# NVIDIA/nv-wavenet

Hardware: AMD Instinct MI355X
Metric: samples/sec (all GPUs) in real time (every utterance >= 24 kHz) and max real-time batch @24kHz, R64/S256/A256 20L fp16 (higher is better)
Workload: dtype f16; 1 GPU; C3: R=64 S=256 A=256 L=20 maxDilation=512 fp16, autoregressive generation at steady state (each step = samples 640..895 of every utterance: all dilated taps live, all rings wrapped; the steps re-run that sample range -- same launch, same memory traffic -- so from the second step on the rings hold the previous step's values: a timing workload, not one long utterance); batch_per_gpu=12288, global_batch=12288, parallelism=batch-sharded x1, final RCCL all_gather

## Files before the change

### include/nv_wavenet_c.h

```cpp
#ifndef NV_WAVENET_C_H
#define NV_WAVENET_C_H

#include <stddef.h>

#ifdef __cplusplus
extern "C" {
#endif

typedef struct nvw_engine nvw_engine;

typedef void (*nvw_consume_fn)(int* yOut, int init_sample, int count, void* user);

#define NVW_ABI_VERSION 7
int nvw_abi_version(void);
int nvw_supported(int R, int S, int A, int precision);
int nvw_list_supported(int* out, int max);

nvw_engine* nvw_create(int R, int S, int A, int precision, int num_layers, int max_dilation,
                       int batch_size, int num_samples, int implementation, int tanh_embed);
nvw_engine* nvw_create_ex(int R, int S, int A, int precision, int num_layers, int max_dilation,
                          int batch_size, int num_samples, int implementation, int tanh_embed,
                          int organisation);
void nvw_destroy(nvw_engine* e);

void nvw_set_embeddings(nvw_engine* e, float* embed_prev, float* embed_cur);
void nvw_set_layer_weights(nvw_engine* e, int layer, float* Wprev, float* Wcur, float* Bh,
                           float* Wres, float* Bres, float* Wskip, float* Bskip);
void nvw_set_out_weights(nvw_engine* e, float* Wzs, float* Bzs, float* Wza, float* Bza);
void nvw_set_inputs(nvw_engine* e, float* Lh, float* output_selectors);

void nvw_set_conditioning(nvw_engine* e, float* Lh);
void nvw_set_inputs_n(nvw_engine* e, float* Lh, float* output_selectors, int num_samples);
void nvw_set_conditioning_n(nvw_engine* e, float* Lh, int num_samples);
void nvw_pack_conditioning(nvw_engine* e, float* Lh, int first_sample, int count, void* stream);
void nvw_set_conditioning_direct(nvw_engine* e, float* Lh, int num_samples);
int nvw_set_conditioning_direct_t(nvw_engine* e, const void* Lh, int num_samples, int precision);
void nvw_set_conditioning_packed(nvw_engine* e, const void* frags, int num_samples);
int nvw_set_conditioning_packed_n(nvw_engine* e, const void* frags, int num_samples, size_t elems);
int nvw_cond_tiles(nvw_engine* e);
int nvw_produce_conditioning_f16(const void* x, const void* wfrag, const float* bias, void* out, int tiles, int num_samples,
                                 int num_layers, int kfrags, int nwf, void* stream);
int nvw_max_cond_channels(void);
int nvw_set_conditioning_weights(nvw_engine* e, const float* Wcond, const float* bcond, int n_cond);
int nvw_feature_fragments(nvw_engine* e);
size_t nvw_feature_elems(nvw_engine* e, int num_samples);
int nvw_set_conditioning_features(nvw_engine* e, const void* frags, int num_samples, size_t elems);
int nvw_pack_features(nvw_engine* e, const void* x, int precision, long long b_stride, long long c_stride, long long t_stride,
                      int first_sample, int count, void* stream);
int nvw_set_features(nvw_engine* e, const void* x, int precision, long long b_stride, long long c_stride, long long t_stride,
                     int num_samples);
int nvw_set_upsampling(nvw_engine* e, const float* up_w, const float* up_b, int window, int stride);
int nvw_set_mel(nvw_engine* e, const void* mel, int precision, long long b_stride, long long c_stride, long long f_stride, int frames);
int nvw_upsample_features(nvw_engine* e, int first_sample, int count, void* stream);
int nvw_get_features(nvw_engine* e, void* dst, int first_sample, int count);
int nvw_generate_stream(nvw_engine* e, int num_samples_per_chunk, nvw_consume_fn consume, void* user, int num_samples, int batch_size, int* yOut,
                        void* stream);
void nvw_set_selectors(nvw_engine* e, float* output_selectors, int num_samples);
unsigned nvw_chain_status(nvw_engine* e);
unsigned nvw_chain_fallbacks(nvw_engine* e);
unsigned nvw_chain_last_timeout(nvw_engine* e);
void nvw_set_chain_timeout_ms(nvw_engine* e, double ms);
void nvw_set_clock_probe(nvw_engine* e, int on);
void nvw_set_ring_in_lds(nvw_engine* e, int mode);
double nvw_last_launch_clock_ghz(nvw_engine* e);
int nvw_run_range(nvw_engine* e, int init_sample, int count, int num_samples, int batch_size, void* stream);
void nvw_reset_history(nvw_engine* e, void* stream);
void nvw_set_selector_seed(nvw_engine* e, unsigned long long seed);
void nvw_set_audio_out(nvw_engine* e, short* pcm_out);
void nvw_set_audio_out_n(nvw_engine* e, short* pcm_out, size_t elems);
void nvw_kernel_info(nvw_engine* e, int batch_size, int dump_activations, char* buf, int buf_size);

int nvw_run(nvw_engine* e, int num_samples, int batch_size, int* yOut, int batch_size_per_block,
            int dump_activations, void* stream);
int nvw_run_partial(nvw_engine* e, int init_sample, int num_samples, int batch_size, int* yOut,
                    int batch_size_per_block, int dump_activations, void* stream);
int nvw_run_chunks(nvw_engine* e, int num_samples_per_chunk, nvw_consume_fn consume, void* user,
                   int num_samples, int batch_size, int* yOut, int batch_size_per_block,
                   int dump_activations, void* stream);

void nvw_get_xt_out(nvw_engine* e, int layer, float* dst);
void nvw_get_skip_out(nvw_engine* e, int layer, float* dst);
void nvw_get_zs(nvw_engine* e, float* dst);
void nvw_get_za(nvw_engine* e, float* dst);
void nvw_get_p(nvw_engine* e, float* dst);
void nvw_get_y_out(nvw_engine* e, int* yOut, int offset, int size, void* stream);

int nvw_slots_begin(nvw_engine* e, int window);
int nvw_slot_start(nvw_engine* e, int slot, const void* x, int precision, long long c_stride, long long t_stride, int length,
                   unsigned uid);
int nvw_slot_stop(nvw_engine* e, int slot);
int nvw_slots_step(nvw_engine* e, int count, int* yOut, short* pcm, void* stream);
void nvw_slots_end(nvw_engine* e);

int nvw_slot_start_mel(nvw_engine* e, int slot, const void* mel, int precision, long long c_stride, long long f_stride, int frames,
                       int final, unsigned uid);
int nvw_slot_mel_frames(nvw_engine* e, int slot, int frames, int final);
int nvw_slots_headroom(nvw_engine* e);
int nvw_slots_get_features(nvw_engine* e, void* dst, long long first_sample, int count);

size_t nvw_slot_state_bytes(nvw_engine* e);
int nvw_slot_move(nvw_engine* e, int from, int to);
int nvw_slot_save(nvw_engine* e, int slot, void* dst, void* stream);
int nvw_slot_resume(nvw_engine* e, int slot, const void* state, const void* x, int precision, long long c_stride, long long t_stride,
                    int length);
int nvw_slot_resume_mel(nvw_engine* e, int slot, const void* state, const void* mel, int precision, long long c_stride,
                        long long f_stride, int frames, int final);

typedef struct {
    int slot;
    unsigned uid;
    int done;
    int mel;
} nvw_slot_saved;
int nvw_slots_save_list(nvw_engine* e, const int* slots, int n, void* dst, long long stride, nvw_slot_saved* saved, void* stream);
typedef struct {
    int slot;
    int mel;
    const void* src;
    int precision;
    long long c_stride, t_stride;
    int length;
    int final;
} nvw_slot_resume_req;
int nvw_slots_resume_list(nvw_engine* e, const nvw_slot_resume_req* reqs, int n, const void* states, long long stride);

typedef struct {
    int slot;
    unsigned uid;
    long long first;
    int n;
    int finished;
    long long offset;
} nvw_slot_piece;
long long nvw_slots_step_ragged(nvw_engine* e, int count, int* samples, short* pcm, long long capacity, nvw_slot_piece* pieces,
                                int max_pieces, int* n_pieces, unsigned long long* ticket, void* stream);
int nvw_slots_wait(nvw_engine* e, unsigned long long ticket);
float nvw_slots_time_outputs(nvw_engine* e, int ragged, int count, int* samples, short* pcm, long long capacity, int reps, void* stream);
int nvw_slots_done(nvw_engine* e, unsigned long long ticket);
void* nvw_pinned_alloc(size_t bytes);
void nvw_pinned_free(void* p);

int nvw_set_temperatures(nvw_engine* e, const float* T, int n);
int nvw_slot_set_temperature(nvw_engine* e, int slot, float T);
float nvw_slot_temperature(nvw_engine* e, int slot);

int nvw_set_prime(nvw_engine* e, const int* y, const int* n, int batch, int max_n, long long stride);
// ... 101 lines not shown
```

### nv_wavenet_amd/_lib.py

```python
import ctypes as C
import os

_HERE = os.path.dirname(os.path.abspath(__file__))
LIB_PATH = os.environ.get("NVW_LIB") or os.path.join(_HERE, "libwavenet_infer.so")

if not os.path.exists(LIB_PATH):
    raise ImportError(
        "nv_wavenet_amd: %s is missing. Build it with `python -c 'import __graft_entry__ as g; g.build()'` "
        "or `make -C nv_wavenet_amd/csrc`. There is no CPU fallback for the engine." % LIB_PATH)

import torch

lib = C.CDLL(LIB_PATH)

_fp = C.c_void_p
CONSUME_FN = C.CFUNCTYPE(None, C.c_void_p, C.c_int, C.c_int, C.c_void_p)

SIGNATURES = {
    "nvw_abi_version": (C.c_int, []),
    "nvw_supported": (C.c_int, [C.c_int] * 4),
    "nvw_list_supported": (C.c_int, [C.POINTER(C.c_int), C.c_int]),
    "nvw_create": (C.c_void_p, [C.c_int] * 10),
    "nvw_create_ex": (C.c_void_p, [C.c_int] * 11),
    "nvw_destroy": (None, [C.c_void_p]),
    "nvw_set_embeddings": (None, [C.c_void_p, _fp, _fp]),
    "nvw_set_layer_weights": (None, [C.c_void_p, C.c_int] + [_fp] * 7),
    "nvw_set_out_weights": (None, [C.c_void_p] + [_fp] * 4),
    "nvw_set_inputs": (None, [C.c_void_p, _fp, _fp]),
    "nvw_set_conditioning": (None, [C.c_void_p, _fp]),
    "nvw_set_inputs_n": (None, [C.c_void_p, _fp, _fp, C.c_int]),
    "nvw_set_conditioning_n": (None, [C.c_void_p, _fp, C.c_int]),
    "nvw_pack_conditioning": (None, [C.c_void_p, _fp, C.c_int, C.c_int, C.c_void_p]),
    "nvw_set_conditioning_direct": (None, [C.c_void_p, _fp, C.c_int]),
    "nvw_set_conditioning_direct_t": (C.c_int, [C.c_void_p, _fp, C.c_int, C.c_int]),
    "nvw_set_conditioning_packed": (None, [C.c_void_p, _fp, C.c_int]),
    "nvw_set_conditioning_packed_n": (C.c_int, [C.c_void_p, _fp, C.c_int, C.c_size_t]),
    "nvw_cond_tiles": (C.c_int, [C.c_void_p]),
    "nvw_produce_conditioning_f16": (C.c_int, [_fp, _fp, _fp, _fp, C.c_int, C.c_int, C.c_int, C.c_int, C.c_int, C.c_void_p]),
    "nvw_max_cond_channels": (C.c_int, []),
    "nvw_set_conditioning_weights": (C.c_int, [C.c_void_p, _fp, _fp, C.c_int]),
    "nvw_feature_fragments": (C.c_int, [C.c_void_p]),
    "nvw_feature_elems": (C.c_size_t, [C.c_void_p, C.c_int]),
    "nvw_set_conditioning_features": (C.c_int, [C.c_void_p, _fp, C.c_int, C.c_size_t]),
    "nvw_pack_features": (C.c_int, [C.c_void_p, _fp, C.c_int, C.c_longlong, C.c_longlong, C.c_longlong, C.c_int, C.c_int, C.c_void_p]),
    "nvw_set_features": (C.c_int, [C.c_void_p, _fp, C.c_int, C.c_longlong, C.c_longlong, C.c_longlong, C.c_int]),
    "nvw_set_upsampling": (C.c_int, [C.c_void_p, _fp, _fp, C.c_int, C.c_int]),
    "nvw_set_mel": (C.c_int, [C.c_void_p, _fp, C.c_int, C.c_longlong, C.c_longlong, C.c_longlong, C.c_int]),
    "nvw_upsample_features": (C.c_int, [C.c_void_p, C.c_int, C.c_int, C.c_void_p]),
    "nvw_get_features": (C.c_int, [C.c_void_p, _fp, C.c_int, C.c_int]),
    "nvw_generate_stream": (C.c_int, [C.c_void_p, C.c_int, CONSUME_FN, C.c_void_p, C.c_int, C.c_int, _fp, C.c_void_p]),
    "nvw_set_selectors": (None, [C.c_void_p, _fp, C.c_int]),
    "nvw_chain_status": (C.c_uint, [C.c_void_p]),
    "nvw_chain_fallbacks": (C.c_uint, [C.c_void_p]),
    "nvw_chain_last_timeout": (C.c_uint, [C.c_void_p]),
    "nvw_set_chain_timeout_ms": (None, [C.c_void_p, C.c_double]),
    "nvw_set_clock_probe": (None, [C.c_void_p, C.c_int]),
    "nvw_set_ring_in_lds": (None, [C.c_void_p, C.c_int]),
    "nvw_last_launch_clock_ghz": (C.c_double, [C.c_void_p]),
    "nvw_run_range": (C.c_int, [C.c_void_p, C.c_int, C.c_int, C.c_int, C.c_int, C.c_void_p]),
    "nvw_reset_history": (None, [C.c_void_p, C.c_void_p]),
    "nvw_set_selector_seed": (None, [C.c_void_p, C.c_ulonglong]),
    "nvw_set_audio_out": (None, [C.c_void_p, C.c_void_p]),
    "nvw_set_audio_out_n": (None, [C.c_void_p, C.c_void_p, C.c_size_t]),
    "nvw_kernel_info": (None, [C.c_void_p, C.c_int, C.c_int, C.c_char_p, C.c_int]),
    "nvw_run": (C.c_int, [C.c_void_p, C.c_int, C.c_int, _fp, C.c_int, C.c_int, C.c_void_p]),
    "nvw_run_partial": (C.c_int, [C.c_void_p, C.c_int, C.c_int, C.c_int, _fp, C.c_int, C.c_int, C.c_void_p]),
    "nvw_run_chunks": (C.c_int, [C.c_void_p, C.c_int, CONSUME_FN, C.c_void_p, C.c_int, C.c_int, _fp, C.c_int,
                                 C.c_int, C.c_void_p]),
    "nvw_get_xt_out": (None, [C.c_void_p, C.c_int, _fp]),
    "nvw_get_skip_out": (None, [C.c_void_p, C.c_int, _fp]),
    "nvw_get_zs": (None, [C.c_void_p, _fp]),
    "nvw_get_za": (None, [C.c_void_p, _fp]),
    "nvw_get_p": (None, [C.c_void_p, _fp]),
    "nvw_get_y_out": (None, [C.c_void_p, _fp, C.c_int, C.c_int, C.c_void_p]),
    "nvw_slots_begin": (C.c_int, [C.c_void_p, C.c_int]),
    "nvw_slot_start": (C.c_int, [C.c_void_p, C.c_int, _fp, C.c_int, C.c_longlong, C.c_longlong, C.c_int, C.c_uint]),
    "nvw_slot_stop": (C.c_int, [C.c_void_p, C.c_int]),
    "nvw_slots_step": (C.c_int, [C.c_void_p, C.c_int, _fp, _fp, C.c_void_p]),
    "nvw_slots_end": (None, [C.c_void_p]),
    "nvw_slot_start_mel": (C.c_int, [C.c_void_p, C.c_int, _fp, C.c_int, C.c_longlong, C.c_longlong, C.c_int, C.c_int, C.c_uint]),
    "nvw_slot_mel_frames": (C.c_int, [C.c_void_p, C.c_int, C.c_int, C.c_int]),
    "nvw_slots_headroom": (C.c_int, [C.c_void_p]),
    "nvw_slots_get_features": (C.c_int, [C.c_void_p, _fp, C.c_longlong, C.c_int]),
    "nvw_slot_state_bytes": (C.c_size_t, [C.c_void_p]),
    "nvw_slot_move": (C.c_int, [C.c_void_p, C.c_int, C.c_int]),
    "nvw_slot_save": (C.c_int, [C.c_void_p, C.c_int, _fp, C.c_void_p]),
    "nvw_slot_resume": (C.c_int, [C.c_void_p, C.c_int, _fp, _fp, C.c_int, C.c_longlong, C.c_longlong, C.c_int]),
    "nvw_slot_resume_mel": (C.c_int, [C.c_void_p, C.c_int, _fp, _fp, C.c_int, C.c_longlong, C.c_longlong, C.c_int, C.c_int]),
    "nvw_slots_save_list": (C.c_int, [C.c_void_p, C.c_void_p, C.c_int, _fp, C.c_longlong, C.c_void_p, C.c_void_p]),
    "nvw_slots_resume_list": (C.c_int, [C.c_void_p, C.c_void_p, C.c_int, _fp, C.c_longlong]),
    "nvw_slots_step_ragged": (C.c_longlong, [C.c_void_p, C.c_int, _fp, _fp, C.c_longlong, C.c_void_p, C.c_int, C.POINTER(C.c_int),
                                             C.POINTER(C.c_ulonglong), C.c_void_p]),
    "nvw_slots_time_outputs": (C.c_float, [C.c_void_p, C.c_int, C.c_int, _fp, _fp, C.c_longlong, C.c_int, C.c_void_p]),
    "nvw_slots_wait": (C.c_int, [C.c_void_p, C.c_ulonglong]),
    "nvw_slots_done": (C.c_int, [C.c_void_p, C.c_ulonglong]),
    "nvw_set_temperatures": (C.c_int, [C.c_void_p, _fp, C.c_int]),
    "nvw_slot_set_temperature": (C.c_int, [C.c_void_p, C.c_int, C.c_float]),
    "nvw_slot_temperature": (C.c_float, [C.c_void_p, C.c_int]),
    "nvw_set_prime": (C.c_int, [C.c_void_p, _fp, _fp, C.c_int, C.c_int, C.c_longlong]),
    "nvw_slot_prime": (C.c_int, [C.c_void_p, C.c_int, _fp, C.c_int]),
    "nvw_slot_primed": (C.c_int, [C.c_void_p, C.c_int]),
    "nvw_prefill_window": (C.c_int, [C.c_void_p]),
    "nvw_prefill_states": (C.c_int, [C.c_void_p, C.c_void_p, C.c_int, _fp, C.c_longlong, C.c_void_p]),
    "nvw_score_max_samples": (C.c_int, [C.c_void_p]),
    "nvw_score_samples": (C.c_int, [C.c_void_p, C.c_void_p, C.c_int, C.c_void_p]),
    "nvw_upsample_row_elems": (C.c_int, [C.c_void_p]),
    "nvw_upsample_requests": (C.c_int, [C.c_void_p, C.c_void_p, C.c_int, C.c_void_p]),
    "nvw_prefill_states_mel": (C.c_int, [C.c_void_p, C.c_void_p, C.c_int, _fp, C.c_longlong, C.c_void_p]),
    "nvw_score_samples_mel": (C.c_int, [C.c_void_p, C.c_void_p, C.c_int, C.c_void_p]),
    "nvw_score_chunks": (C.c_int, [C.c_void_p, C.c_void_p, C.c_int, C.c_void_p]),
    "nvw_score_chunks_mel": (C.c_int, [C.c_void_p, C.c_void_p, C.c_int, C.c_void_p]),
    "nvw_pinned_alloc": (C.c_void_p, [C.c_size_t]),
    "nvw_pinned_free": (None, [C.c_void_p]),
    "nvw_device_synchronize": (None, []),
    "nvw_time_runs": (C.c_float, [C.c_void_p, C.c_int, C.c_int, C.c_int, C.c_int, C.c_void_p]),
    "wavenet_infer": (None, [C.c_int, C.c_int, _fp, _fp, C.c_int, C.c_int] + [C.POINTER(C.c_void_p)] * 7 +
                      [_fp, _fp, C.c_int, _fp, C.c_int, _fp]),
    "get_R": (C.c_int, []),
    "get_S": (C.c_int, []),
    "get_A": (C.c_int, []),
}

ABI_VERSION = 7
_abi = getattr(lib, "nvw_abi_version", None)
_have = None
if _abi is not None:
    _abi.restype, _abi.argtypes = C.c_int, []
    _have = _abi()
if _have != ABI_VERSION:
    raise ImportError("nv_wavenet_amd: %s implements revision %s of include/nv_wavenet_c.h, this package expects %d: rebuild it "
                      "(make -C nv_wavenet_amd/csrc)" % (LIB_PATH, "<none: too old>" if _have is None else _have, ABI_VERSION))

for _name, (_res, _args) in SIGNATURES.items():
    _fn = getattr(lib, _name)
    _fn.restype = _res
    _fn.argtypes = _args


def addr(x):
    if x is None:
# ... 11 lines not shown
```

### nv_wavenet_amd/csrc/engine_base.hpp

```cpp
#pragma once
#include "../../include/nv_wavenet_c.h"
#include "nv_wavenet.hpp"

struct nvw_engine {
    virtual ~nvw_engine() {}
    virtual void setEmbeddings(float*, float*) = 0;
    virtual void setLayerWeights(int, float*, float*, float*, float*, float*, float*, float*) = 0;
    virtual void setOutWeights(float*, float*, float*, float*) = 0;
    virtual void setInputs(float*, float*, int) = 0;
    virtual void setConditioning(float*, int) = 0;
    virtual void packConditioning(float*, int, int, hipStream_t) = 0;
    virtual void setConditioningDirect(const void*, int, int) = 0;
    virtual void setConditioningPacked(const void*, int) = 0;
    virtual int condTiles() = 0;
    virtual bool setConditioningWeights(const float*, const float*, int) = 0;
    virtual int featureFragments() = 0;
    virtual size_t featureElems(int) = 0;
    virtual void setConditioningFeatures(const void*, int) = 0;
    virtual void packFeatures(const void*, int, long long, long long, long long, int, int, hipStream_t) = 0;
    virtual void setFeatures(const void*, int, long long, long long, long long, int) = 0;
    virtual int conditioningChannels() = 0;
    virtual bool setUpsampling(const float*, const float*, int, int) = 0;
    virtual int upsamplingStride() = 0;
    virtual int melSamples() = 0;
    virtual bool hasFeatureBuffer() = 0;
    virtual int maxBatch() = 0;
    virtual void getFeatures(void*, int, int) = 0;
    virtual void setMel(const void*, int, long long, long long, long long, int) = 0;
    virtual void upsampleFeatures(int, int, hipStream_t) = 0;
    virtual bool run_stream(int, nvw_consume_fn, void*, int, int, int*, hipStream_t) = 0;
    virtual size_t condPackedElems(int) = 0;
    virtual void setSelectors(float*, int) = 0;
    virtual bool run_range(int, int, int, int, hipStream_t) = 0;
    virtual void resetHistory(hipStream_t) = 0;
    virtual bool supported() = 0;
    virtual unsigned chainStatus() = 0;
    virtual unsigned chainFallbacks() = 0;
    virtual unsigned chainLastTimeout() = 0;
    virtual void setChainTimeoutMs(double) = 0;
    virtual void setClockProbe(bool) = 0;
    virtual void setRingInLds(int) = 0;
    virtual double lastLaunchClockGHz() = 0;
    virtual int precisionBits() = 0;
    virtual int maxSamples() = 0;
    virtual void setSelectorSeed(unsigned long long) = 0;
    virtual void setAudioOut(short*, size_t) = 0;
    virtual void kernelInfo(int, bool, char*, int) = 0;
    virtual bool run(int, int, int*, int, bool, hipStream_t) = 0;
    virtual bool run_partial(int, int, int, int*, int, bool, hipStream_t) = 0;
    virtual bool run_chunks(int, nvw_consume_fn, void*, int, int, int*, int, bool, hipStream_t) = 0;
    virtual void getXtOut(int, float*) = 0;
    virtual void getSkipOut(int, float*) = 0;
    virtual void getZs(float*) = 0;
    virtual void getZa(float*) = 0;
    virtual void getP(float*) = 0;
    virtual void getYOut(int*, int, int, hipStream_t) = 0;
    virtual bool setTemperatures(const float*, int) = 0;
    virtual bool setPrime(const int*, const int*, int, int, long long) = 0;
    virtual int prefillWindow() = 0;
    virtual int prefillStates(const wn::PrefillReq*, int, void*, long long, hipStream_t) = 0;
    virtual int scoreMaxSamples() = 0;
    virtual int scoreSamples(const wn::ScoreReq*, int, hipStream_t) = 0;
    virtual int upsampleRowElems() = 0;
    virtual int upsampleRequests(const wn::MelTimeReq*, int, hipStream_t) = 0;
    virtual int prefillStatesMel(const wn::PrefillMelReq*, int, void*, long long, hipStream_t) = 0;
    virtual int scoreSamplesMel(const wn::ScoreMelReq*, int, hipStream_t) = 0;
    virtual int scoreChunks(const wn::ScoreChunkReq*, int, hipStream_t) = 0;
    virtual int scoreChunksMel(const wn::ScoreChunkMelReq*, int, hipStream_t) = 0;
    virtual wn::SlotSession& slots() = 0;
};
static_assert(sizeof(nvw_slot_piece) == sizeof(wn::SlotPiece) && offsetof(nvw_slot_piece, slot) == offsetof(wn::SlotPiece, slot) &&
              offsetof(nvw_slot_piece, uid) == offsetof(wn::SlotPiece, uid) && offsetof(nvw_slot_piece, finished) == offsetof(wn::SlotPiece, finished) &&
              offsetof(nvw_slot_piece, first) == offsetof(wn::SlotPiece, first) &&
              offsetof(nvw_slot_piece, n) == offsetof(wn::SlotPiece, n) && offsetof(nvw_slot_piece, offset) == offsetof(wn::SlotPiece, offset),
              "nvw_slot_piece is wn::SlotPiece");

static_assert(sizeof(nvw_slot_saved) == sizeof(wn::SlotSaved) && offsetof(nvw_slot_saved, slot) == offsetof(wn::SlotSaved, slot) &&
              offsetof(nvw_slot_saved, uid) == offsetof(wn::SlotSaved, uid) && offsetof(nvw_slot_saved, done) == offsetof(wn::SlotSaved, done) &&
              offsetof(nvw_slot_saved, mel) == offsetof(wn::SlotSaved, mel),
              "nvw_slot_saved is wn::SlotSaved");
static_assert(sizeof(nvw_slot_resume_req) == sizeof(wn::SlotResumeReq) && offsetof(nvw_slot_resume_req, slot) == offsetof(wn::SlotResumeReq, slot) &&
              offsetof(nvw_slot_resume_req, mel) == offsetof(wn::SlotResumeReq, mel) && offsetof(nvw_slot_resume_req, src) == offsetof(wn::SlotResumeReq, src) &&
              offsetof(nvw_slot_resume_req, precision) == offsetof(wn::SlotResumeReq, precision) &&
              offsetof(nvw_slot_resume_req, c_stride) == offsetof(wn::SlotResumeReq, cStride) &&
              offsetof(nvw_slot_resume_req, t_stride) == offsetof(wn::SlotResumeReq, tStride) &&
              offsetof(nvw_slot_resume_req, length) == offsetof(wn::SlotResumeReq, length) &&
              offsetof(nvw_slot_resume_req, final) == offsetof(wn::SlotResumeReq, final),
              "nvw_slot_resume_req is wn::SlotResumeReq");

static_assert(sizeof(nvw_prefill_req) == sizeof(wn::PrefillReq) && offsetof(nvw_prefill_req, y) == offsetof(wn::PrefillReq, y) &&
              offsetof(nvw_prefill_req, n) == offsetof(wn::PrefillReq, n) && offsetof(nvw_prefill_req, x) == offsetof(wn::PrefillReq, x) &&
              offsetof(nvw_prefill_req, precision) == offsetof(wn::PrefillReq, precision) &&
              offsetof(nvw_prefill_req, c_stride) == offsetof(wn::PrefillReq, cStride) &&
              offsetof(nvw_prefill_req, t_stride) == offsetof(wn::PrefillReq, tStride) && offsetof(nvw_prefill_req, uid) == offsetof(wn::PrefillReq, uid) &&
              offsetof(nvw_prefill_req, temperature) == offsetof(wn::PrefillReq, temperature),
              "nvw_prefill_req is wn::PrefillReq");

static_assert(sizeof(nvw_score_req) == sizeof(wn::ScoreReq) && offsetof(nvw_score_req, y) == offsetof(wn::ScoreReq, y) &&
              offsetof(nvw_score_req, n) == offsetof(wn::ScoreReq, n) && offsetof(nvw_score_req, x) == offsetof(wn::ScoreReq, x) &&
              offsetof(nvw_score_req, precision) == offsetof(wn::ScoreReq, precision) &&
              offsetof(nvw_score_req, c_stride) == offsetof(wn::ScoreReq, cStride) &&
              offsetof(nvw_score_req, t_stride) == offsetof(wn::ScoreReq, tStride) &&
              offsetof(nvw_score_req, temperature) == offsetof(wn::ScoreReq, temperature) &&
              offsetof(nvw_score_req, logp) == offsetof(wn::ScoreReq, logp) && offsetof(nvw_score_req, rows) == offsetof(wn::ScoreReq, rows),
              "nvw_score_req is wn::ScoreReq");
static_assert(sizeof(nvw_upsample_req) == sizeof(wn::MelTimeReq) && offsetof(nvw_upsample_req, mel) == offsetof(wn::MelTimeReq, mel) &&
              offsetof(nvw_upsample_req, precision) == offsetof(wn::MelTimeReq, precision) &&
              offsetof(nvw_upsample_req, c_stride) == offsetof(wn::MelTimeReq, cStride) &&
              offsetof(nvw_upsample_req, f_stride) == offsetof(wn::MelTimeReq, fStride) &&
              offsetof(nvw_upsample_req, frames) == offsetof(wn::MelTimeReq, frames) &&
              offsetof(nvw_upsample_req, first_sample) == offsetof(wn::MelTimeReq, first) &&
              offsetof(nvw_upsample_req, count) == offsetof(wn::MelTimeReq, count) && offsetof(nvw_upsample_req, dst) == offsetof(wn::MelTimeReq, dst),
              "nvw_upsample_req is wn::MelTimeReq");
static_assert(sizeof(nvw_prefill_mel_req) == sizeof(wn::PrefillMelReq) && offsetof(nvw_prefill_mel_req, y) == offsetof(wn::PrefillMelReq, y) &&
              offsetof(nvw_prefill_mel_req, n) == offsetof(wn::PrefillMelReq, n) && offsetof(nvw_prefill_mel_req, mel) == offsetof(wn::PrefillMelReq, mel) &&
              offsetof(nvw_prefill_mel_req, precision) == offsetof(wn::PrefillMelReq, precision) &&
              offsetof(nvw_prefill_mel_req, c_stride) == offsetof(wn::PrefillMelReq, cStride) &&
              offsetof(nvw_prefill_mel_req, f_stride) == offsetof(wn::PrefillMelReq, fStride) &&
              offsetof(nvw_prefill_mel_req, frames) == offsetof(wn::PrefillMelReq, frames) &&
              offsetof(nvw_prefill_mel_req, uid) == offsetof(wn::PrefillMelReq, uid) &&
              offsetof(nvw_prefill_mel_req, temperature) == offsetof(wn::PrefillMelReq, temperature),
              "nvw_prefill_mel_req is wn::PrefillMelReq");
static_assert(sizeof(nvw_score_mel_req) == sizeof(wn::ScoreMelReq) && offsetof(nvw_score_mel_req, y) == offsetof(wn::ScoreMelReq, y) &&
              offsetof(nvw_score_mel_req, n) == offsetof(wn::ScoreMelReq, n) && offsetof(nvw_score_mel_req, mel) == offsetof(wn::ScoreMelReq, mel) &&
              offsetof(nvw_score_mel_req, precision) == offsetof(wn::ScoreMelReq, precision) &&
              offsetof(nvw_score_mel_req, c_stride) == offsetof(wn::ScoreMelReq, cStride) &&
              offsetof(nvw_score_mel_req, f_stride) == offsetof(wn::ScoreMelReq, fStride) &&
              offsetof(nvw_score_mel_req, frames) == offsetof(wn::ScoreMelReq, frames) &&
              offsetof(nvw_score_mel_req, temperature) == offsetof(wn::ScoreMelReq, temperature) &&
              offsetof(nvw_score_mel_req, logp) == offsetof(wn::ScoreMelReq, logp) && offsetof(nvw_score_mel_req, rows) == offsetof(wn::ScoreMelReq, rows),
              "nvw_score_mel_req is wn::ScoreMelReq");
static_assert(sizeof(nvw_score_chunk_req) == sizeof(wn::ScoreChunkReq) && offsetof(nvw_score_chunk_req, state) == offsetof(wn::ScoreChunkReq, state) &&
              offsetof(nvw_score_chunk_req, y) == offsetof(wn::ScoreChunkReq, y) && offsetof(nvw_score_chunk_req, n) == offsetof(wn::ScoreChunkReq, n) &&
              offsetof(nvw_score_chunk_req, x) == offsetof(wn::ScoreChunkReq, x) &&
              offsetof(nvw_score_chunk_req, precision) == offsetof(wn::ScoreChunkReq, precision) &&
              offsetof(nvw_score_chunk_req, c_stride) == offsetof(wn::ScoreChunkReq, cStride) &&
              offsetof(nvw_score_chunk_req, t_stride) == offsetof(wn::ScoreChunkReq, tStride) &&
              offsetof(nvw_score_chunk_req, uid) == offsetof(wn::ScoreChunkReq, uid) &&
              offsetof(nvw_score_chunk_req, temperature) == offsetof(wn::ScoreChunkReq, temperature) &&
              offsetof(nvw_score_chunk_req, logp) == offsetof(wn::ScoreChunkReq, logp) &&
              offsetof(nvw_score_chunk_req, rows) == offsetof(wn::ScoreChunkReq, rows) &&
              offsetof(nvw_score_chunk_req, state_out) == offsetof(wn::ScoreChunkReq, stateOut),
              "nvw_score_chunk_req is wn::ScoreChunkReq");
static_assert(sizeof(nvw_score_chunk_mel_req) == sizeof(wn::ScoreChunkMelReq) &&
              offsetof(nvw_score_chunk_mel_req, state) == offsetof(wn::ScoreChunkMelReq, state) &&
              offsetof(nvw_score_chunk_mel_req, y) == offsetof(wn::ScoreChunkMelReq, y) &&
              offsetof(nvw_score_chunk_mel_req, n) == offsetof(wn::ScoreChunkMelReq, n) &&
              offsetof(nvw_score_chunk_mel_req, mel) == offsetof(wn::ScoreChunkMelReq, mel) &&
              offsetof(nvw_score_chunk_mel_req, precision) == offsetof(wn::ScoreChunkMelReq, precision) &&
              offsetof(nvw_score_chunk_mel_req, c_stride) == offsetof(wn::ScoreChunkMelReq, cStride) &&
              offsetof(nvw_score_chunk_mel_req, f_stride) == offsetof(wn::ScoreChunkMelReq, fStride) &&
              offsetof(nvw_score_chunk_mel_req, frames) == offsetof(wn::ScoreChunkMelReq, frames) &&
              offsetof(nvw_score_chunk_mel_req, uid) == offsetof(wn::ScoreChunkMelReq, uid) &&
              offsetof(nvw_score_chunk_mel_req, temperature) == offsetof(wn::ScoreChunkMelReq, temperature) &&
              offsetof(nvw_score_chunk_mel_req, logp) == offsetof(wn::ScoreChunkMelReq, logp) &&
              offsetof(nvw_score_chunk_mel_req, rows) == offsetof(wn::ScoreChunkMelReq, rows) &&
              offsetof(nvw_score_chunk_mel_req, state_out) == offsetof(wn::ScoreChunkMelReq, stateOut),
              "nvw_score_chunk_mel_req is wn::ScoreChunkMelReq");

template <typename Tw, typename Td, int R, int S, int A>
struct EngineImpl : nvw_engine {
    nvWavenetInfer<Tw, Td, R, S, A> eng;
    int cap;
    EngineImpl(int L, int maxD, int B, int N, int impl, bool tanhEmbed, int org) : eng(L, maxD, B, N, impl, tanhEmbed, org), cap(N) {}
    void setEmbeddings(float* p, float* c) override { eng.setEmbeddings(p, c); }
    void setLayerWeights(int l, float* a, float* b, float* c, float* d, float* e, float* f, float* g) override {
        eng.setLayerWeights(l, a, b, c, d, e, f, g);
    }
    void setOutWeights(float* a, float* b, float* c, float* d) override { eng.setOutWeights(a, b, c, d); }
    void setInputs(float* Lh, float* sel, int n) override { eng.setInputs(Lh, sel, n); }
    void setConditioning(float* Lh, int n) override { eng.setConditioning(Lh, n); }
    void packConditioning(float* Lh, int first, int count, hipStream_t s) override { eng.packConditioning(Lh, first, count, s); }
    void setConditioningDirect(const void* Lh, int n, int prec) override { eng.setConditioningDirect(Lh, n, prec); }
    void setConditioningPacked(const void* frags, int n) override { eng.setConditioningPacked(frags, n); }
    int condTiles() override { return eng.condTiles(); }
    bool setConditioningWeights(const float* W, const float* b, int n) override { return eng.setConditioningWeights(W, b, n); }
    int featureFragments() override { return eng.featureFragments(); }
    size_t featureElems(int n) override { return eng.featureElems(n); }
    void setConditioningFeatures(const void* f, int n) override { eng.setConditioningFeatures(f, n); }
    void packFeatures(const void* x, int prec, long long bS, long long cS, long long tS, int first, int count, hipStream_t s) override {
        eng.packFeatures(x, prec, bS, cS, tS, first, count, s);
    }
    void setFeatures(const void* x, int prec, long long bS, long long cS, long long tS, int n) override { eng.setFeatures(x, prec, bS, cS, tS, n); }
    int conditioningChannels() override { return eng.conditioningChannels(); }
    bool setUpsampling(const float* W, const float* b, int window, int stride) override { return eng.setUpsampling(W, b, window, stride); }
    int upsamplingStride() override { return eng.upsamplingStride(); }
    int melSamples() override { return eng.melSamples(); }
    bool hasFeatureBuffer() override { return eng.hasFeatureBuffer(); }
    int maxBatch() override { return eng.maxBatch(); }
    void getFeatures(void* d, int first, int count) override { eng.getFeatures(d, first, count); }
    void setMel(const void* mel, int prec, long long bS, long long cS, long long fS, int frames) override { eng.setMel(mel, prec, bS, cS, fS, frames); }
    void upsampleFeatures(int first, int count, hipStream_t s) override { eng.upsampleFeatures(first, count, s); }
    bool run_stream(int chunk, nvw_consume_fn fn, void* user, int n, int b, int* y, hipStream_t s) override {
        return eng.run_stream(chunk, [fn, user](int* yo, int i, int c) { if (fn) fn(yo, i, c, user); }, n, b, y, s);
    }
    size_t condPackedElems(int n) override { return eng.condPackedElems(n); }
    void setSelectors(float* sel, int n) override { eng.setSelectors(sel, n); }
    bool run_range(int i, int c, int n, int b, hipStream_t s) override { return eng.run_range(i, c, n, b, s); }
    void resetHistory(hipStream_t s) override { eng.resetHistory(s); }
    bool supported() override { return eng.supported(); }
    unsigned chainStatus() override { return eng.chainStatus(); }
    unsigned chainFallbacks() override { return eng.chainFallbacks(); }
    unsigned chainLastTimeout() override { return eng.chainLastTimeout(); }
    void setChainTimeoutMs(double ms) override { eng.setChainTimeoutMs(ms); }
    void setClockProbe(bool on) override { eng.setClockProbe(on); }
    void setRingInLds(int mode) override { eng.setRingInLds(mode); }
    double lastLaunchClockGHz() override { return eng.lastLaunchClockGHz(); }
    int precisionBits() override { return std::is_same<Td, float>::value ? 32 : 16; }
    int maxSamples() override { return cap; }
    void setSelectorSeed(unsigned long long seed) override { eng.setSelectorSeed(seed); }
    void setAudioOut(short* pcm, size_t n) override { eng.setAudioOut(pcm, n); }
    void kernelInfo(int b, bool dump, char* buf, int n) override { eng.kernelInfo(b, dump, buf, n); }
    bool run(int n, int b, int* y, int bspb, bool dump, hipStream_t s) override {
        return eng.run(n, b, y, bspb, dump, s);
    }
    bool run_partial(int i, int n, int b, int* y, int bspb, bool dump, hipStream_t s) override {
        return eng.run_partial(i, n, b, y, bspb, dump, s);
    }
    bool run_chunks(int chunk, nvw_consume_fn fn, void* user, int n, int b, int* y, int bspb, bool dump,
                    hipStream_t s) override {
        return eng.run_chunks(chunk, [fn, user](int* yo, int i, int c) { if (fn) fn(yo, i, c, user); }, n, b, y,
                              bspb, dump, s);
    }
    void getXtOut(int l, float* d) override { eng.getXtOut(l, d); }
    void getSkipOut(int l, float* d) override { eng.getSkipOut(l, d); }
    void getZs(float* d) override { eng.getZs(d); }
    void getZa(float* d) override { eng.getZa(d); }
    void getP(float* d) override { eng.getP(d); }
    void getYOut(int* y, int off, int size, hipStream_t s) override { eng.getYOut(y, off, size, s); }
    bool setTemperatures(const float* T, int n) override { return eng.setTemperatures(T, n); }
    bool setPrime(const int* y, const int* n, int batch, int maxN, long long stride) override { return eng.setPrime(y, n, batch, maxN, stride); }
    int prefillWindow() override { return eng.prefillWindow(); }
    int prefillStates(const wn::PrefillReq* reqs, int count, void* dst, long long stride, hipStream_t s) override {
        return eng.prefillStates(reqs, count, dst, stride, s);
    }
    int scoreMaxSamples() override { return eng.scoreMaxSamples(); }
    int scoreSamples(const wn::ScoreReq* reqs, int count, hipStream_t s) override { return eng.scoreSamples(reqs, count, s); }
    int upsampleRowElems() override { return eng.upsampleRowElems(); }
    int upsampleRequests(const wn::MelTimeReq* reqs, int count, hipStream_t s) override { return eng.upsampleRequests(reqs, count, s); }
    int prefillStatesMel(const wn::PrefillMelReq* reqs, int count, void* dst, long long stride, hipStream_t s) override {
        return eng.prefillStatesMel(reqs, count, dst, stride, s);
    }
    int scoreSamplesMel(const wn::ScoreMelReq* reqs, int count, hipStream_t s) override { return eng.scoreSamplesMel(reqs, count, s); }
    int scoreChunks(const wn::ScoreChunkReq* reqs, int count, hipStream_t s) override { return eng.scoreChunks(reqs, count, s); }
    int scoreChunksMel(const wn::ScoreChunkMelReq* reqs, int count, hipStream_t s) override { return eng.scoreChunksMel(reqs, count, s); }
    wn::SlotSession& slots() override { return eng.slots(); }
};

typedef nvw_engine* (*nvw_factory_fn)(int L, int maxD, int B, int N, int impl, int tanhEmbed, int organisation);

#define WN_CAT2(a, b) a##b
#define WN_CAT(a, b) WN_CAT2(a, b)
#define WN_FACTORY_NAME(R, S, A, P) WN_CAT(WN_CAT(WN_CAT(WN_CAT(WN_CAT(WN_CAT(WN_CAT(nvw_make_, R), _), S), _), A), _p), P)
```

### nv_wavenet_amd/csrc/nv_wavenet.hpp

```cpp
#pragma once

#include <assert.h>
#include <hip/hip_fp16.h>
#include <hip/hip_runtime.h>
#include <stdio.h>
#include <stdlib.h>
#include <string.h>

#include <cmath>
#include <memory>
#include <type_traits>
#include <vector>

#include "gpu_check.hpp"
#include "mel_time.hpp"
#include "prefill.hpp"
#include "score.hpp"
#include "score_carry.hpp"
#include "slots_session.hpp"
#include "wn_chain.hpp"
#include "wn_kernels.hpp"

enum nvwOrganisation {
    NVW_ORG_AUTO = 0,
    NVW_ORG_WG = 1,
    NVW_ORG_WG1 = 2,
    NVW_ORG_WG2 = 3,
    NVW_ORG_WG3 = 4,
    NVW_ORG_CHAIN = 5,
    NVW_ORG_CHAIN1 = 6,
    NVW_ORG_RETIRED7 = 7,
    NVW_ORG_RETIRED8 = 8,
    NVW_ORG_RETIRED9 = 9,
    NVW_ORG_WG4 = 10,
    NVW_ORG_LAST = NVW_ORG_WG4
};

template <typename T_weight, typename T_data, int R = 64, int S = 128, int A = 256>
class nvWavenetInfer : protected wn::SlotHost {
public:
    enum Implementation { AUTO = 0, SINGLE_BLOCK, DUAL_BLOCK, PERSISTENT, MANYBLOCK_NONPERSISTENT };

    static constexpr bool F16 = !std::is_same<T_data, float>::value;
    static_assert(std::is_same<T_data, float>::value || std::is_same<T_data, half>::value,
                  "T_data must be float or half");
    static_assert(std::is_same<T_weight, float>::value == std::is_same<T_data, float>::value,
                  "T_weight/T_data must be <float,float> or <half2,half>");

protected:
    using C = wn::Cfg<F16, R, S, A, 1>;
    using CC = wn::CCfg<F16, R, S, A>;
    using elem = typename wn::Prec<F16>::elem;
    static constexpr int KFC = wn::feat_kfc<F16>();
    static constexpr int KC = KFC * 16 * wn::Prec<F16>::TPF;
    using CF = wn::Cfg<F16, R, S, A, 1, KFC>;
    static_assert(wn::kSoftScaleUnit == wn::kLog2e, "T = 1 is the kernel's default scale");

    Implementation m_implementation;
    int m_numLayers, m_maxBatch, m_maxSamples, m_maxDilation, m_tiles, m_numCUs;
    int m_org;
    bool m_supported;
    int m_chainLpc, m_chainStages;
    bool m_tanhEmbed;
    int m_num_samples_per_chunk;
    int m_ringSlots;
    int m_ringDirtyTiles;
    int m_ringLdsMode;
    int m_lastStride;

    elem* m_wblob;
    float* m_bias;
    elem* m_embedPrev;
    elem* m_embedCur;
    elem* m_cond;
    int m_condRawSamples;
    const void* m_condRaw;
    int m_condRawKind;
    const void* m_condUser;
    int m_condUserSamples;
    elem* m_wblobF;
    float* m_biasF;
    float* m_condW;
    float* m_condB;
    int2* m_restream;
    int m_restreamN;
    int m_nCond;
    bool m_featDirty;
    elem* m_upTab;
    float* m_upBias;
    int m_upWindow, m_upStride;
    elem* m_melFrag;
    int m_melFrames, m_melCap;
    elem* m_feat;
    const void* m_featPtr;
    int m_featSamples;
    float* m_outputSelectors;
    elem* m_ring;
    int *m_yInPrev, *m_yInCur, *m_yOut;
    float *m_XtOut, *m_skipOut, *m_Zs, *m_Za, *m_p;
    unsigned long long* m_mail;
    unsigned* m_chainStatus;
    size_t m_mailBytes;
    elem* m_ringShadow;
    int* m_histShadow;
    long long m_chainTimeoutTicks;

    float* m_stage;
    size_t m_stageElems;

    bool m_useRng;
    unsigned long long m_rngSeed;
    short* m_pcm;
    short* m_mulaw;
    short* m_pcmUser;
    size_t m_pcmUserElems;
    unsigned long long* m_clk;
    bool m_clkOn;

    wn::TemperatureTable m_temps;
    wn::PrimeTable m_prime;
    wn::Score m_score;
    wn::MelTime m_melTime;
    wn::Prefill m_prefill;
    std::unique_ptr<wn::SlotSession> m_slots;

    std::vector<hipEvent_t> m_poolEvents;
    hipEvent_t pooledEvent(size_t i) {
        while (m_poolEvents.size() <= i) {
            hipEvent_t ev;
            gpuErrChk(hipEventCreateWithFlags(&ev, hipEventDisableTiming));
            m_poolEvents.push_back(ev);
        }
        return m_poolEvents[i];
    }
    static bool isDevicePtr(const void* ptr) { return wn::is_device_ptr(ptr); }
    size_t m_stageUsed;
    void stageBegin(size_t totalElems) {
        if (totalElems > m_stageElems) {
            gpuErrChk(hipStreamSynchronize(0));
            if (m_stage) gpuErrChk(hipFree(m_stage));
            gpuErrChk(hipMalloc(&m_stage, totalElems * sizeof(float)));
            m_stageElems = totalElems;
        }
        m_stageUsed = 0;
    }
    const float* onDevice(const float* src, size_t n) {
        if (isDevicePtr(src)) return src;
        assert(m_stageUsed + n <= m_stageElems);
        float* d = m_stage + m_stageUsed;
        m_stageUsed += (n + 3) & ~(size_t)3;
        gpuErrChk(hipMemcpyAsync(d, src, n * sizeof(float), hipMemcpyHostToDevice, 0));
        return d;
    }
    static int gridFor(size_t n) {
        size_t g = (n + 255) / 256;
        return (int)(g > 4096 ? 4096 : (g ? g : 1));
    }
    void packWeight(size_t blockFrag, const float* src, int M, int K, int gateRT) {
        const float* d = onDevice(src, (size_t)M * K);
        hipLaunchKernelGGL((wn::pack_weight_kernel<F16>), dim3(gridFor((size_t)M * K)), dim3(256), 0, 0,
                           m_wblob + blockFrag * C::FRAG_ELEMS, d, M, K, C::NW,
                           C::waveStreamFrags(m_numLayers) * C::FRAG_ELEMS, gateRT);
        gpuErrChk(hipGetLastError());
    }
    void convertTo(elem* dst, const float* src, size_t n) {
        const float* d = onDevice(src, n);
        hipLaunchKernelGGL((wn::convert_kernel<F16>), dim3(gridFor(n)), dim3(256), 0, 0, dst, d, n);
        gpuErrChk(hipGetLastError());
    }
    template <int BT> static size_t ldsNeed(int L, int embTables, bool dump = true) { return wn::Cfg<F16, R, S, A, BT>::ldsBytes(L, embTables, dump); }
    static constexpr size_t kLdsMax = 160 * 1024;
    template <int BT> bool ldsFits(bool dump = true) const { return ldsNeed<BT>(m_numLayers, 0, dump) <= kLdsMax; }
    template <int BT> int embTables(bool dump = true) const {
        return ldsNeed<BT>(m_numLayers, 2, dump) <= kLdsMax ? 2 : ldsNeed<BT>(m_numLayers, 1, dump) <= kLdsMax ? 1 : 0;
    }
    void fillSchedule(wn::Params& p) const {
        int d = 1, off = 0;
        for (int l = 0; l < m_numLayers; l++) {
            p.dil[l].d = d;
            p.dil[l].off = off;
            p.dil[l].lds = 0;
            off += d;
            d <<= 1;
            if (d > m_maxDilation) d = 1;
        }
        p.dil[m_numLayers] = p.dil[0];
        p.dil[m_numLayers + 1] = p.dil[1];
    }
    template <int BT> size_t placeLdsRing(wn::Params& p, size_t need) const {
        using CB = wn::Cfg<F16, R, S, A, BT>;
        int D = 0;
        for (int d = 1; d <= m_maxDilation && d <= WN_LDS_RING_MAXD; d <<= 1)
            if (need + (size_t)CB::ringTailSlots(CB::ldsRingSlots(m_numLayers, m_maxDilation, d)) * CB::RING_SLOT <= kLdsMax) D = d;
        p.ldsRingD = D;
        int slot = 0;
        for (int l = 0; l < m_numLayers; l++) {
            p.dil[l].lds = slot;
            if (p.dil[l].d <= D) slot += p.dil[l].d;
        }
        p.dil[m_numLayers] = p.dil[0];
        p.dil[m_numLayers + 1] = p.dil[1];
        return (size_t)CB::ringTailSlots(slot) * CB::RING_SLOT;
    }
    static constexpr bool lrBuilt(bool dump, int raw) { return !dump && (raw == 0 || F16); }
    template <int BT> size_t ringPlan(wn::Params& p, size_t need, bool dump, int raw) const {
        p.ldsRingD = 0;
#ifdef WN_EXP_TWO_WG
        if (BT == 1) return 0;
#endif
        if (!lrBuilt(dump, raw) || m_ringLdsMode < 0) return 0;
        wn::Params q = p;
        const size_t bytes = placeLdsRing<BT>(q, need);
        if (q.ldsRingD <= 0) return 0;
        p = q;
        return bytes;
    }
    template <int BT, bool EMB, bool DUMP, int RAW> bool launchK(wn::Params& p, int tiles, int nEmb, hipStream_t stream) {
        using CB = wn::Cfg<F16, R, S, A, BT>;
        const int grid = (tiles + BT - 1) / BT;
        p.embLds = nEmb;
        const size_t need = ldsNeed<BT>(m_numLayers, nEmb, DUMP);
        if constexpr (lrBuilt(DUMP, RAW)) {
            const size_t ringBytes = ringPlan<BT>(p, need, DUMP, RAW);
            if (p.ldsRingD > 0) {
                hipLaunchKernelGGL((wn::wavenet_wg<F16, R, S, A, BT, EMB, DUMP, RAW, true>), dim3(grid), dim3(CB::THREADS), need + ringBytes, stream, p);
                return hipGetLastError() == hipSuccess;
            }
        }
        p.ldsRingD = 0;
        hipLaunchKernelGGL((wn::wavenet_wg<F16, R, S, A, BT, EMB, DUMP, RAW>), dim3(grid), dim3(CB::THREADS), need, stream, p);
        return hipGetLastError() == hipSuccess;
    }
    template <int BT> int planEmb(bool dump, int raw) const {
        int nEmb = embTables<BT>(dump);
#ifdef WN_EXP_TWO_WG
        if (BT == 1) return 0;
#endif
        if (nEmb == 2 && m_ringLdsMode >= 0 && lrBuilt(dump, raw)) {
            wn::Params q;
            fillSchedule(q);
            placeLdsRing<BT>(q, ldsNeed<BT>(m_numLayers, 2, dump));
            const int D2 = q.ldsRingD;
            placeLdsRing<BT>(q, ldsNeed<BT>(m_numLayers, 1, dump));
            if (D2 == 0 || (D2 < 2 && q.ldsRingD > D2)) nEmb = 1;
        }
        return nEmb;
    }
    template <int BT, bool DUMP, int RAW> bool launchE(wn::Params& p, int tiles, hipStream_t stream) {
        const int nEmb = planEmb<BT>(DUMP, RAW);
        return nEmb ? launchK<BT, true, DUMP, RAW>(p, tiles, nEmb, stream) : launchK<BT, false, DUMP, RAW>(p, tiles, 0, stream);
    }
    template <int BT, bool DUMP> bool launchD(wn::Params& p, int tiles, hipStream_t stream) {
        if (p.condRawKind == 3) return launchE<BT, DUMP, 3>(p, tiles, stream);
        if constexpr (F16) {
            if (p.condRawKind == 2) return launchE<BT, DUMP, 2>(p, tiles, stream);
        }
        return p.condRawKind == 1 ? launchE<BT, DUMP, 1>(p, tiles, stream) : launchE<BT, DUMP, 0>(p, tiles, stream);
    }
    template <int BT> bool launch(wn::Params& p, int tiles, hipStream_t stream) {
        if (!p.dump) {
            if constexpr (F16) return launchD<BT, false>(p, tiles, stream);
            else if (p.condRawKind == 0) return launchE<BT, false, 0>(p, tiles, stream);
        }
        return launchD<BT, true>(p, tiles, stream);
    }
    template <int BT, bool EMB, bool DUMP, int RAW> void allowLdsK() {
        const size_t need = ldsNeed<BT>(m_numLayers, EMB ? embTables<BT>(DUMP) : 0, DUMP);
        if (need <= kLdsMax) {
            gpuErrChk(hipFuncSetAttribute((const void*)wn::wavenet_wg<F16, R, S, A, BT, EMB, DUMP, RAW>,
                                          hipFuncAttributeMaxDynamicSharedMemorySize, (int)need));
            if constexpr (lrBuilt(DUMP, RAW))
                gpuErrChk(hipFuncSetAttribute((const void*)wn::wavenet_wg<F16, R, S, A, BT, EMB, DUMP, RAW, true>,
                                              hipFuncAttributeMaxDynamicSharedMemorySize, (int)kLdsMax));
        }
    }
    template <int BT, bool DUMP> void allowLdsD() {
        allowLdsK<BT, false, DUMP, 0>();
        allowLdsK<BT, true, DUMP, 0>();
        allowLdsK<BT, false, DUMP, 1>();
        allowLdsK<BT, true, DUMP, 1>();
        allowLdsK<BT, false, DUMP, 3>();
        allowLdsK<BT, true, DUMP, 3>();
        if constexpr (F16) {
            allowLdsK<BT, false, DUMP, 2>();
            allowLdsK<BT, true, DUMP, 2>();
        }
    }
    template <int BT> void allowLds() {
        allowLdsD<BT, true>();
        if constexpr (F16) allowLdsD<BT, false>();
        else {
            allowLdsK<BT, false, false, 0>();
            allowLdsK<BT, true, false, 0>();
        }
    }
    float* headBias() { return m_bias + (size_t)m_numLayers * C::BIAS_L; }

    static int chainStagesFor(int L, int lpc) { return (L + lpc - 1) / lpc + 1; }
    static int chainLpcMax(int L) {
        if (!CC::SUPPORTED) return 0;
        const int ns = (L + CC::LPC - 1) / CC::LPC;
        return (L + ns - 1) / ns;
    }
    bool chainFits(int lpc, int tiles) const {
        return lpc > 0 && chainStagesFor(m_numLayers, lpc) * ((tiles + CC::TPC_MAX - 1) / CC::TPC_MAX) <= m_numCUs;
    }
    int singleOrg(int) const { return NVW_ORG_WG; }
    struct OrgTimes {
        static constexpr double kClockMHz = 2390.0;
        static constexpr double kStreamBytesPerClk = 58.0;
        static constexpr double kStreamLayerUs = 0.25;
        static constexpr double kHeadUs = 4.0;
        static constexpr double kChainHopUs = 1.1;
        static constexpr double kChainLayerUs(int r) { return r >= 128 ? 0.55 : 0.4; }
        static constexpr double kChainUnitUs = 5.0;
    };
    int pickOrganisation(int tiles) const {
        const int single = singleOrg(tiles);
        const int lpc = chainLpcMax(m_numLayers);
        if (!chainFits(lpc, tiles)) return single;
        const double wBytes = sizeof(elem) * ((double)m_numLayers * (5.0 * R * R + (double)S * R) + (double)A * S + (double)A * A);
        const int wgMax = WG3 ? 3 : WG2 ? 2 : 1;
        const int rounds = (tiles + wgMax * m_numCUs - 1) / (wgMax * m_numCUs);
        const double tStream = (wBytes / (OrgTimes::kStreamBytesPerClk * OrgTimes::kClockMHz) + OrgTimes::kStreamLayerUs * m_numLayers + OrgTimes::kHeadUs) * rounds;
        const int stages = chainStagesFor(m_numLayers, lpc), perLaunch = m_numCUs / stages;
        const int tpc = (tiles + perLaunch - 1) / perLaunch;
        if (tpc > 1 && WG3) return single;
        double tChain = OrgTimes::kChainHopUs * stages + OrgTimes::kChainLayerUs(R) * m_numLayers + OrgTimes::kHeadUs;
        if (tpc * OrgTimes::kChainUnitUs > tChain) tChain = tpc * OrgTimes::kChainUnitUs;
        const double tWg = tiles > m_numCUs ? tStream * (tiles > 2 * m_numCUs && WG3 ? 1.9 : WG2 ? 1.4 : 1.0) : tStream;
        return tChain < tWg ? NVW_ORG_CHAIN : single;
    }
    void resolveOrganisation(int requested) {
        const int tiles = (m_maxBatch + 15) / 16;
        int org = requested;
        if (org == NVW_ORG_AUTO) {
            switch (m_implementation) {
                case SINGLE_BLOCK: org = singleOrg(tiles); break;
                case DUAL_BLOCK:
                case PERSISTENT: org = chainFits(chainLpcMax(m_numLayers), tiles) ? NVW_ORG_CHAIN : singleOrg(tiles); break;
                case MANYBLOCK_NONPERSISTENT:
                    org = (CC::SUPPORTED && chainFits(1, tiles)) ? NVW_ORG_CHAIN1
                          : chainFits(chainLpcMax(m_numLayers), tiles) ? NVW_ORG_CHAIN : singleOrg(tiles);
                    break;
                default: org = pickOrganisation(tiles); break;
            }
        }
        if (org == NVW_ORG_CHAIN && !chainFits(chainLpcMax(m_numLayers), tiles)) org = singleOrg(tiles);
        if (org == NVW_ORG_CHAIN1 && !(CC::SUPPORTED && chainFits(1, tiles))) org = singleOrg(tiles);
        m_org = org;
        m_chainLpc = org == NVW_ORG_CHAIN ? chainLpcMax(m_numLayers) : org == NVW_ORG_CHAIN1 ? 1 : 0;
        m_chainStages = m_chainLpc ? chainStagesFor(m_numLayers, m_chainLpc) : 0;
    }
    bool isChain() const { return m_chainLpc > 0; }
    static constexpr bool kChainHoistBuilt = F16 && CC::SUPPORTED && CC::LP <= 2 && A <= 512;
    static bool chainHoists(int tpc) { return kChainHoistBuilt && tpc > WN_CHAIN_HOIST_FROM; }
    int chainTpc(int tiles) const {
        const int perLaunch = m_numCUs / (m_chainStages > 0 ? m_chainStages : 1);
        int tpc = perLaunch > 0 ? (tiles + perLaunch - 1) / perLaunch : 1;
#ifdef WN_CHAIN_TPC_MIN
        if (tpc < WN_CHAIN_TPC_MIN) tpc = WN_CHAIN_TPC_MIN;
#endif
        return tpc < 1 ? 1 : tpc > CC::TPC_MAX ? CC::TPC_MAX : tpc;
    }
    static constexpr bool WG3 = F16 && R <= 64;
    static constexpr bool WG2 = R < 128;
    bool wg3Fits() const {
        if constexpr (WG3) return ldsFits<3>();
        return false;
    }
    static constexpr bool WG4 = WG3;
    bool wg4Fits() const {
        if constexpr (WG4) return ldsFits<4>(false);
        return false;
    }
    int wgTiles(int tiles) const {
#ifdef WN_EXP_TWO_WG
        if (m_org == NVW_ORG_WG && tiles <= 2 * m_numCUs) return 1;
#endif
        bool four = m_org == NVW_ORG_WG4;
        if (m_org == NVW_ORG_WG && tiles > WN_WG4_FROM * m_numCUs) {
            const int r4 = (tiles + 4 * m_numCUs - 1) / (4 * m_numCUs), r3 = (tiles + 3 * m_numCUs - 1) / (3 * m_numCUs);
            four = r4 * 47 <= r3 * 36;
        }
        if (four && wg4Fits() && wg3Fits()) return 4;
        const bool three = four || m_org == NVW_ORG_WG3 || (m_org == NVW_ORG_WG && tiles > 2 * m_numCUs);
        if (three && wg3Fits()) return 3;
        const bool two = three || m_org == NVW_ORG_WG2 || (m_org == NVW_ORG_WG && tiles > m_numCUs);
        if constexpr (WG2) return (two && ldsFits<2>()) ? 2 : 1;
        return 1;
    }

public:
    nvWavenetInfer(int numLayers, int maxDilation, int batchSize, int numSamples, int impl = 0,
                   bool tanhEmbed = true, int organisation = NVW_ORG_AUTO)
        : m_implementation((Implementation)impl), m_numLayers(numLayers), m_maxBatch(batchSize),
          m_maxSamples(numSamples), m_maxDilation(maxDilation), m_tanhEmbed(tanhEmbed),
          m_num_samples_per_chunk(0), m_lastStride(numSamples), m_cond(NULL), m_condRawSamples(0), m_condRaw(NULL), m_condRawKind(0), m_condUser(NULL), m_condUserSamples(0),
          m_wblobF(NULL), m_biasF(NULL), m_condW(NULL), m_condB(NULL), m_restream(NULL), m_restreamN(0), m_nCond(0), m_featDirty(true),
          m_upTab(NULL), m_upBias(NULL), m_upWindow(0), m_upStride(0), m_melFrag(NULL), m_melFrames(0), m_melCap(0),
          m_feat(NULL), m_featPtr(NULL), m_featSamples(0),
          m_mail(NULL), m_chainStatus(NULL), m_mailBytes(0), m_ringShadow(NULL), m_histShadow(NULL),
          m_chainTimeoutTicks(wn::kChainTimeoutTicks), m_stage(NULL), m_stageElems(0), m_useRng(false), m_rngSeed(0), m_pcm(NULL),
          m_mulaw(NULL), m_pcmUser(NULL), m_pcmUserElems(0), m_clk(NULL), m_clkOn(false), m_temps(batchSize), m_prime(batchSize), m_stageUsed(0) {
        assert(numLayers >= 2 && batchSize > 0 && numSamples > 0 && maxDilation > 0);
        m_ringDirtyTiles = 0;
        m_ringLdsMode = 0;
        assert(numLayers <= wn::kMaxLayers);
        {
            int dev = 0;
            hipDeviceProp_t prop;
            gpuErrChk(hipGetDevice(&dev));
            gpuErrChk(hipGetDeviceProperties(&prop, dev));
            m_numCUs = prop.multiProcessorCount;
        }
        resolveOrganisation(organisation);
        m_supported = isChain() || ldsFits<1>();
        if (!m_supported)
            fprintf(stderr, "nvWavenetInfer: R=%d S=%d A=%d with %d layers needs %zu bytes of LDS (> 160 KiB): unsupported\n", R,
                    S, A, numLayers, ldsNeed<1>(numLayers, 0));

        {
            const int tiles = (batchSize + 15) / 16;
            int group = isChain() ? 1 : wgTiles(tiles);
            if (group >= 3 && wg4Fits()) group = 12;
            m_tiles = (tiles + group - 1) / group * group;
        }

        {
            int d = 1, slots = 0;
            for (int l = 0; l < numLayers; l++) {
                slots += d;
                d <<= 1;
                if (d > maxDilation) d = 1;
            }
            m_ringSlots = slots;
        }

        const size_t wElems = (size_t)C::NW * C::waveStreamFrags(numLayers) * C::FRAG_ELEMS;
        gpuErrChk(hipMalloc(&m_wblob, wElems * sizeof(elem)));
        gpuErrChk(hipMemset(m_wblob, 0, wElems * sizeof(elem)));
        const size_t bElems = (size_t)numLayers * C::BIAS_L + 2 * A;
        gpuErrChk(hipMalloc(&m_bias, bElems * sizeof(float)));
        gpuErrChk(hipMemset(m_bias, 0, bElems * sizeof(float)));
        gpuErrChk(hipMalloc(&m_embedPrev, (size_t)A * R * sizeof(elem)));
        gpuErrChk(hipMalloc(&m_embedCur, (size_t)A * R * sizeof(elem)));
        gpuErrChk(hipMemset(m_embedPrev, 0, (size_t)A * R * sizeof(elem)));
        gpuErrChk(hipMemset(m_embedCur, 0, (size_t)A * R * sizeof(elem)));

        gpuErrChk(hipMalloc(&m_outputSelectors, (size_t)numSamples * batchSize * sizeof(float)));
        gpuErrChk(hipMemset(m_outputSelectors, 0, (size_t)numSamples * batchSize * sizeof(float)));

        const size_t ringBytes = ringElems() * sizeof(elem);
        gpuErrChk(hipMalloc(&m_ring, ringBytes));
        gpuErrChk(hipMemset(m_ring, 0, ringBytes));

        gpuErrChk(hipMalloc(&m_yInPrev, batchSize * sizeof(int)));
        gpuErrChk(hipMalloc(&m_yInCur, batchSize * sizeof(int)));
        gpuErrChk(hipMalloc(&m_yOut, (size_t)numSamples * batchSize * sizeof(int)));
        gpuErrChk(hipMemset(m_yOut, 0, (size_t)numSamples * batchSize * sizeof(int)));

        gpuErrChk(hipMalloc(&m_XtOut, (size_t)numLayers * R * batchSize * sizeof(float)));
        gpuErrChk(hipMalloc(&m_skipOut, (size_t)numLayers * S * batchSize * sizeof(float)));
        gpuErrChk(hipMalloc(&m_Zs, (size_t)A * batchSize * sizeof(float)));
        gpuErrChk(hipMalloc(&m_Za, (size_t)A * batchSize * sizeof(float)));
        gpuErrChk(hipMalloc(&m_p, (size_t)A * batchSize * sizeof(float)));
        gpuErrChk(hipMemset(m_XtOut, 0, (size_t)numLayers * R * batchSize * sizeof(float)));
        gpuErrChk(hipMemset(m_skipOut, 0, (size_t)numLayers * S * batchSize * sizeof(float)));
        gpuErrChk(hipMemset(m_Zs, 0, (size_t)A * batchSize * sizeof(float)));
        gpuErrChk(hipMemset(m_Za, 0, (size_t)A * batchSize * sizeof(float)));
        gpuErrChk(hipMemset(m_p, 0, (size_t)A * batchSize * sizeof(float)));

        gpuErrChk(hipMalloc(&m_chainStatus, 4 * sizeof(unsigned)));
        gpuErrChk(hipMemset(m_chainStatus, 0, 4 * sizeof(unsigned)));
        if (isChain()) {
            {
                const int tiles = (batchSize + 15) / 16, perLaunch = m_numCUs / m_chainStages;
                m_mailBytes = CC::mailGranules(tiles < perLaunch ? tiles : perLaunch, m_chainStages, chainTpc(tiles)) * sizeof(unsigned long long);
            }
            gpuErrChk(hipMalloc(&m_mail, m_mailBytes));
            gpuErrChk(hipMemset(m_mail, 0, m_mailBytes));
            gpuErrChk(hipFuncSetAttribute((const void*)wn::wavenet_chain<F16, R, S, A, true>,
                                          hipFuncAttributeMaxDynamicSharedMemorySize, (int)CC::ldsBytes()));
            gpuErrChk(hipFuncSetAttribute((const void*)wn::wavenet_chain<F16, R, S, A, false>,
                                          hipFuncAttributeMaxDynamicSharedMemorySize, (int)CC::ldsBytes()));
            if constexpr (kChainHoistBuilt)
                gpuErrChk(hipFuncSetAttribute((const void*)wn::wavenet_chain<F16, R, S, A, false, true>,
                                              hipFuncAttributeMaxDynamicSharedMemorySize, (int)CC::ldsBytes()));
            if (chainHasFallback()) {
                gpuErrChk(hipMalloc(&m_ringShadow, ringBytes));
// ... 4 lines not shown
        hipLaunchKernelGGL(wn::silence_kernel, dim3(1), dim3(256), 0, 0, m_yInPrev, m_yInCur, m_maxBatch);
        gpuErrChk(hipGetLastError());

        if (ldsFits<1>()) {
            allowLds<1>();
            if (!isChain()) {
                if constexpr (WG2) allowLds<2>();
                if constexpr (WG3) allowLds<3>();
                if constexpr (WG4) {
                    if (wg4Fits()) {
                        allowLdsK<4, false, false, 0>();
                        allowLdsK<4, true, false, 0>();
                    }
                }
            }
        }
        gpuErrChk(hipDeviceSynchronize());
        m_slots.reset(new wn::SlotSession(wn::SlotFacts{m_maxBatch, m_tiles, m_numLayers, m_maxDilation, m_ringSlots, (int)(R * 16 * sizeof(elem) / 1024), R,
                                                        F16, featureElems(1), m_supported, m_ring, m_yInPrev, m_yInCur, A},
                                          *this, m_temps));
    }

    virtual ~nvWavenetInfer() {
        gpuErrChk(hipDeviceSynchronize());
        m_slots.reset();
        for (hipEvent_t ev : m_poolEvents) gpuErrChk(hipEventDestroy(ev));
        gpuErrChk(hipFree(m_wblob));
        gpuErrChk(hipFree(m_bias));
        gpuErrChk(hipFree(m_embedPrev));
        gpuErrChk(hipFree(m_embedCur));
        if (m_cond) gpuErrChk(hipFree(m_cond));
        if (m_wblobF) gpuErrChk(hipFree(m_wblobF));
        if (m_biasF) gpuErrChk(hipFree(m_biasF));
        if (m_condW) gpuErrChk(hipFree(m_condW));
        if (m_condB) gpuErrChk(hipFree(m_condB));
        if (m_restream) gpuErrChk(hipFree(m_restream));
        if (m_feat) gpuErrChk(hipFree(m_feat));
        if (m_upTab) gpuErrChk(hipFree(m_upTab));
        if (m_upBias) gpuErrChk(hipFree(m_upBias));
        if (m_melFrag) gpuErrChk(hipFree(m_melFrag));
        gpuErrChk(hipFree(m_outputSelectors));
        gpuErrChk(hipFree(m_ring));
        gpuErrChk(hipFree(m_yInPrev));
        gpuErrChk(hipFree(m_yInCur));
        gpuErrChk(hipFree(m_yOut));
        gpuErrChk(hipFree(m_XtOut));
        gpuErrChk(hipFree(m_skipOut));
        gpuErrChk(hipFree(m_Zs));
        gpuErrChk(hipFree(m_Za));
        gpuErrChk(hipFree(m_p));
        gpuErrChk(hipFree(m_chainStatus));
        if (m_mail) gpuErrChk(hipFree(m_mail));
        if (m_ringShadow) gpuErrChk(hipFree(m_ringShadow));
        if (m_histShadow) gpuErrChk(hipFree(m_histShadow));
        if (m_stage) gpuErrChk(hipFree(m_stage));
        if (m_pcm) gpuErrChk(hipFree(m_pcm));
        if (m_mulaw) gpuErrChk(hipFree(m_mulaw));
        if (m_clk) gpuErrChk(hipFree(m_clk));
    }

    bool supported() const { return m_supported; }
    unsigned chainStatus() { return statusWord(0); }
    unsigned chainFallbacks() { return statusWord(2); }
    unsigned chainLastTimeout() { return statusWord(1); }
    void setClockProbe(bool on) {
        if (on && !m_clk) {
            gpuErrChk(hipMalloc(&m_clk, 4 * sizeof(unsigned long long)));
            gpuErrChk(hipMemset(m_clk, 0, 4 * sizeof(unsigned long long)));
        }
        m_clkOn = on;
    }
    double lastLaunchClockGHz() {
        if (!m_clk) return 0.0;
        unsigned long long c[4];
        gpuErrChk(hipDeviceSynchronize());
        gpuErrChk(hipMemcpy(c, m_clk, sizeof(c), hipMemcpyDeviceToHost));
        int dev = 0, wallKHz = 0;
        gpuErrChk(hipGetDevice(&dev));
        gpuErrChk(hipDeviceGetAttribute(&wallKHz, hipDeviceAttributeWallClockRate, dev));
        if (c[3] <= c[1] || wallKHz <= 0) return 0.0;
        return (double)(c[2] - c[0]) / (double)(c[3] - c[1]) * (double)wallKHz * 1e-6;
    }
    void setRingInLds(int mode) { m_ringLdsMode = mode < 0 ? -1 : 0; }
    void setChainTimeoutMs(double ms) { m_chainTimeoutTicks = (long long)(ms * 1e5); }

    virtual void setEmbeddings(float* embedPrev, float* embedCur) {
        stageBegin((size_t)2 * A * R);
        convertTo(m_embedPrev, embedPrev, (size_t)A * R);
        convertTo(m_embedCur, embedCur, (size_t)A * R);
        gpuErrChk(hipStreamSynchronize(0));
    }
    bool setConditioningWeights(const float* Wcond, const float* bcond, int nCond) {
        if (nCond <= 0 || nCond > wn::kCondChannelsMax) return false;
        const size_t nW = (size_t)m_numLayers * 2 * R * nCond, nB = (size_t)m_numLayers * 2 * R;
        stageBegin(nW + nB + 8);
        if (!m_condW) {
            gpuErrChk(hipMalloc(&m_condW, (size_t)m_numLayers * KC * 2 * R * sizeof(float)));
            gpuErrChk(hipMalloc(&m_condB, nB * sizeof(float)));
        }
        gpuErrChk(hipMemsetAsync(m_condW, 0, (size_t)m_numLayers * KC * 2 * R * sizeof(float), 0));
        const float* dW = onDevice(Wcond, nW);
        hipLaunchKernelGGL(wn::cond_weight_arrange_kernel, dim3(gridFor(nW)), dim3(256), 0, 0, m_condW, dW, m_numLayers, 2 * R, nCond, KC);
        gpuErrChk(hipGetLastError());
        gpuErrChk(hipMemcpyAsync(m_condB, bcond, nB * sizeof(float), hipMemcpyDefault, 0));
        gpuErrChk(hipStreamSynchronize(0));
        if (nCond != m_nCond) {
            m_upStride = 0;
            m_upWindow = 0;
            m_melFrames = 0;
        }
        m_nCond = nCond;
        m_featDirty = true;
        return true;
    }
    int conditioningChannels() const { return m_nCond; }
    int featureFragments() const { return KFC; }
    size_t featureElems(int numSamples) const { return (size_t)numSamples * m_tiles * KFC * C::FRAG_ELEMS; }
    void setConditioningFeatures(const void* frags, int numSamples) {
        assert(numSamples > 0 && numSamples <= m_maxSamples && m_nCond > 0);
        assert(isDevicePtr(frags));
        resetHistory(0);
        gpuErrChk(hipStreamSynchronize(0));
        dropLhConditioning();
        m_featPtr = frags;
        m_featSamples = numSamples;
    }
    void packFeatures(const void* x, int precision, long long bStride, long long cStride, long long tStride, int firstSample, int count,
                      hipStream_t stream = 0) {
        assert(firstSample >= 0 && count > 0 && firstSample + count <= m_maxSamples && m_nCond > 0);
        assert(precision == 32 || precision == 16);
        assert(isDevicePtr(x));
        if (!m_feat) {
            gpuErrChk(hipMalloc(&m_feat, featureElems(m_maxSamples) * sizeof(elem)));
            gpuErrChk(hipMemsetAsync(m_feat, 0, featureElems(m_maxSamples) * sizeof(elem), stream));
            gpuErrChk(hipStreamSynchronize(stream));
        }
        dropLhConditioning();
        m_featPtr = m_feat;
        m_featSamples = m_maxSamples;
        const int tilesUsed = (m_maxBatch + 15) / 16;
        const size_t nblk = (size_t)tilesUsed * ((count + 7) / 8);
        hipLaunchKernelGGL((wn::pack_features_kernel<F16>), dim3((unsigned)(nblk > 65536 ? 65536 : nblk)), dim3(256), 0, stream,
                           m_feat + featureElems(firstSample), x, precision, bStride, cStride, tStride, m_nCond, m_maxBatch, count, m_tiles,
                           tilesUsed);
        gpuErrChk(hipGetLastError());
    }
    void setFeatures(const void* x, int precision, long long bStride, long long cStride, long long tStride, int numSamples) {
        resetHistory(0);
        packFeatures(x, precision, bStride, cStride, tStride, 0, numSamples, 0);
        gpuErrChk(hipStreamSynchronize(0));
    }
    bool conditioningFromFeatures() const { return m_featPtr != NULL; }
    static constexpr int kUpMaxTaps = 5;
    bool setUpsampling(const float* upW, const float* upB, int window, int stride) {
        if (m_nCond <= 0 || stride <= 0 || window < stride || window % stride != 0 || window / stride > kUpMaxTaps) return false;
        const size_t nW = (size_t)m_nCond * m_nCond * window;
        stageBegin(nW + 128);
        if (m_upTab) gpuErrChk(hipFree(m_upTab));
        const size_t tabElems = (size_t)stride * wn::kUpRowTiles * (window / stride) * KFC * C::FRAG_ELEMS;
        gpuErrChk(hipMalloc(&m_upTab, tabElems * sizeof(elem)));
        if (!m_upBias) gpuErrChk(hipMalloc(&m_upBias, wn::kUpRowTiles * 16 * sizeof(float)));
        gpuErrChk(hipMemsetAsync(m_upBias, 0, wn::kUpRowTiles * 16 * sizeof(float), 0));
        const float* dW = onDevice(upW, nW);
        hipLaunchKernelGGL((wn::pack_upsample_kernel<F16>), dim3(gridFor(tabElems)), dim3(256), 0, 0, m_upTab, dW, m_nCond, window, stride);
        gpuErrChk(hipGetLastError());
        gpuErrChk(hipMemcpyAsync(m_upBias, upB, m_nCond * sizeof(float), hipMemcpyDefault, 0));
// ... 216 lines not shown
    }
    void setSelectorSeed(unsigned long long seed) {
        m_useRng = true;
        m_rngSeed = seed;
    }
    void setAudioOut(short* pcmOut, size_t pcmElems = 0) {
        m_pcmUser = pcmOut;
        m_pcmUserElems = pcmOut ? pcmElems : 0;
        if (pcmOut && !m_pcm) {
            gpuErrChk(hipMalloc(&m_pcm, (size_t)m_maxSamples * m_maxBatch * sizeof(short)));
            gpuErrChk(hipMemset(m_pcm, 0, (size_t)m_maxSamples * m_maxBatch * sizeof(short)));
            ensureMulaw();
        }
    }
    void ensureMulaw() {
        if (!m_mulaw) {
            std::vector<short> table(A);
            const double mu = (double)A - 1.0;
            for (int y = 0; y < A; y++) {
                const double signal = 2.0 * ((double)y / mu) - 1.0;
                const double magnitude = (1.0 / mu) * (std::pow(1.0 + mu, std::fabs(signal)) - 1.0);
                const double v = 32768.0 * (signal > 0 ? magnitude : (signal < 0 ? -magnitude : 0.0));
                table[y] = (short)(int)v;
            }
            gpuErrChk(hipMalloc(&m_mulaw, A * sizeof(short)));
            gpuErrChk(hipMemcpy(m_mulaw, table.data(), A * sizeof(short), hipMemcpyHostToDevice));
        }
    }
    void getAudioOut(short* pcm, int offset, int size, hipStream_t stream = 0) {
        gpuErrChk(hipMemcpy2DAsync(pcm + offset, m_lastStride * sizeof(short), m_pcm + offset,
                                   m_lastStride * sizeof(short), size * sizeof(short), m_maxBatch, hipMemcpyDefault,
                                   stream));
    }

    void kernelInfo(int batch_size, bool dumpActivations, char* buf, int n) const {
        const int tiles = (batch_size + 15) / 16;
        const bool feat = m_featPtr != NULL || m_slots->active();
        const bool chainLaunch = isChain() && !feat;
        const bool dump = dumpActivations || (!F16 && !chainLaunch && (feat || m_condRaw));
        if (chainLaunch) {
            const int perLaunch = m_numCUs / m_chainStages, chains = tiles < perLaunch ? tiles : perLaunch;
            const int tpcNow = chainTpc((m_maxBatch + 15) / 16);
            snprintf(buf, n, "wn::wavenet_chain<%s,%d,%d,%d,DUMP=%d%s> stages=%d layers/stage=%d chains=%d tiles/chain=%d wgs=%d lds=%zu",
                     F16 ? "fp16" : "fp32", R, S, A, dump ? 1 : 0, (!dump && chainHoists(tpcNow)) ? ",HOIST=1" : "", m_chainStages, m_chainLpc, chains, tpcNow,
                     m_chainStages * chains, CC::ldsBytes());
            return;
        }
        const int raw = feat ? 3 : m_condRaw ? m_condRawKind : 0;
        const int bt = launchTiles(tiles, dump, raw);
        int nEmb = planEmb<1>(dump, raw);
        size_t lds = ldsNeed<1>(m_numLayers, nEmb, dump);
        if constexpr (WG2) {
            if (bt == 2) {
                nEmb = planEmb<2>(dump, raw);
                lds = ldsNeed<2>(m_numLayers, nEmb, dump);
            }
        }
        if constexpr (WG3) {
            if (bt == 3) {
                nEmb = planEmb<3>(dump, raw);
                lds = ldsNeed<3>(m_numLayers, nEmb, dump);
            }
            if (bt == 4) {
                nEmb = planEmb<4>(dump, raw);
                lds = ldsNeed<4>(m_numLayers, nEmb, dump);
            }
        }
        int ringD = 0;
        {
            wn::Params q;
            fillSchedule(q);
            size_t rb = 0;
            if (bt == 1) rb = ringPlan<1>(q, lds, dump, raw);
            if constexpr (WG2) {
                if (bt == 2) rb = ringPlan<2>(q, lds, dump, raw);
            }
            if constexpr (WG3) {
                if (bt == 3) rb = ringPlan<3>(q, lds, dump, raw);
                if (bt == 4) rb = ringPlan<4>(q, lds, dump, raw);
            }
            lds += rb;
            ringD = q.ldsRingD;
        }
        char ring[48] = "";
        if (ringD > 0) snprintf(ring, sizeof(ring), " ring_in_lds=d<=%d", ringD);
        snprintf(buf, n, "wn::wavenet_wg<%s,%d,%d,%d,BT=%d,EMBLDS=%d,DUMP=%d,RAW=%d%s> tiles/wg=%d wgs=%d lds=%zu%s",
                 F16 ? "fp16" : "fp32", R, S, A, bt, nEmb, dump ? 1 : 0, raw, ringD > 0 ? ",LR=1" : "", bt, (tiles + bt - 1) / bt, lds, ring);
    }

    void getXtOut(int layer, float* hXt) {
        gpuErrChk(hipMemcpy(hXt, m_XtOut + (size_t)layer * m_maxBatch * R, (size_t)m_maxBatch * R * sizeof(float),
                            hipMemcpyDefault));
    }
    void getSkipOut(int layer, float* hSkipOut) {
        gpuErrChk(hipMemcpy(hSkipOut, m_skipOut + (size_t)layer * m_maxBatch * S,
                            (size_t)m_maxBatch * S * sizeof(float), hipMemcpyDefault));
    }
    void getZs(float* hZs) { gpuErrChk(hipMemcpy(hZs, m_Zs, (size_t)m_maxBatch * A * sizeof(float), hipMemcpyDefault)); }
    void getZa(float* hZa) { gpuErrChk(hipMemcpy(hZa, m_Za, (size_t)m_maxBatch * A * sizeof(float), hipMemcpyDefault)); }
    void getP(float* hP) { gpuErrChk(hipMemcpy(hP, m_p, (size_t)m_maxBatch * A * sizeof(float), hipMemcpyDefault)); }
    void getYOut(int* yOut, int offset, int size, hipStream_t stream = 0) {
        const size_t rowBytes = (size_t)m_lastStride * sizeof(int);
        gpuErrChk(hipMemcpy2DAsync(yOut + offset, rowBytes, m_yOut + offset, rowBytes, (size_t)size * sizeof(int),
                                   (size_t)m_maxBatch, hipMemcpyDefault, stream));
    }

    bool setTemperatures(const float* T, int n) {
        if (m_slots->active()) return false;
        if (T != NULL) {
            if (n < 1 || n > m_maxBatch) return false;
            for (int b = 0; b < n; b++)
                if (!wn::temperature_ok(T[b])) return false;
        }
        gpuErrChk(hipDeviceSynchronize());
        m_temps.reset(false);
        if (T == NULL) return true;
        for (int b = 0; b < n; b++) m_temps.set(b, T[b]);
        m_temps.upload();
        return true;
    }
    float temperature(int b) const { return m_temps.get(b); }

    bool setPrime(const int* y, const int* n, int batch, int maxN, long long stride) {
        if (m_slots->active()) return false;
        if (y == NULL) {
            gpuErrChk(hipDeviceSynchronize());
            m_prime.clear();
            return true;
        }
        if (n == NULL || batch < 1 || batch > m_maxBatch || maxN < 0 || maxN > m_maxSamples || stride < maxN) return false;
        for (int b = 0; b < batch; b++)
            if (n[b] < 0 || n[b] > maxN) return false;
        if (!isDevicePtr(y))
            for (int b = 0; b < batch; b++)
                for (int k = 0; k < n[b]; k++)
                    if (y[b * stride + k] < 0 || y[b * stride + k] >= A) return false;
        m_prime.set(y, n, batch, maxN, stride, m_maxSamples);
        return true;
    }
    int prefillWindow() const { return m_nCond > 0 ? wn::prefill_window(m_ringSlots) : 0; }
    int prefillStates(const wn::PrefillReq* reqs, int count, void* dst, long long stride, hipStream_t stream = 0) {
        if (m_nCond <= 0 || !m_supported) return 0;
        wn::PrefillModel m = prefillModel();
        if (m_featDirty) buildFeatStream(stream);
        m.wblob = m_wblobF;
        m.bias = m_biasF;
        return m_prefill.run(m, reqs, count, dst, stride, stream) ? count : 0;
    }
    wn::PrefillModel prefillModel() const {
        const int L = m_numLayers;
        wn::PrefillModel m;
        m.f16 = F16;
        m.R = R;
        m.A = A;
        m.numLayers = L;
        m.maxDilation = m_maxDilation;
        m.ringSlots = m_ringSlots;
        m.nCond = m_nCond;
        m.tanhEmbed = m_tanhEmbed ? 1 : 0;
        m.wblob = NULL;
        m.waveStreamFrags = CF::waveStreamFrags(L);
        m.bias = NULL;
        m.biasL = C::BIAS_L;
        m.embPrev = m_embedPrev;
        m.embCur = m_embedCur;
        for (int l = 0, d = 1, off = 0; l < L; l++) {
            int dN = d << 1;
            if (dN > m_maxDilation) dN = 1;
// ... 537 lines not shown
```

### nv_wavenet_amd/csrc/wavenet_capi.hip

```cpp
#include <stdlib.h>

#include <vector>

#include "../../include/wavenet_infer.h"
#include "engine_base.hpp"

#define X(R, S, A, P) nvw_engine* WN_FACTORY_NAME(R, S, A, P)(int, int, int, int, int, int, int);
WN_INSTANCES
#undef X

namespace {
struct Entry { int R, S, A, P; nvw_factory_fn make; };
#define X(R, S, A, P) {R, S, A, P, WN_FACTORY_NAME(R, S, A, P)},
const Entry kEntries[] = {WN_INSTANCES};
#undef X
const int kNumEntries = sizeof(kEntries) / sizeof(kEntries[0]);

const Entry* findEntry(int R, int S, int A, int P) {
    for (int i = 0; i < kNumEntries; i++)
        if (kEntries[i].R == R && kEntries[i].S == S && kEntries[i].A == A && kEntries[i].P == P) return &kEntries[i];
    return NULL;
}
}

// ... 119 lines not shown
        fprintf(stderr, "nvw_set_conditioning_features: %zu elements cannot hold %d samples of feature fragments (%zu needed)\n", elems,
                num_samples, e->featureElems(num_samples));
        return 0;
    }
    e->setConditioningFeatures(frags, num_samples);
    return 1;
}
int nvw_pack_features(nvw_engine* e, const void* x, int precision, long long b_stride, long long c_stride, long long t_stride,
                      int first_sample, int count, void* stream) {
    if (!featArgsOk(e, "nvw_pack_features", x, first_sample, count) || (precision != 32 && precision != 16)) return 0;
    e->packFeatures(x, precision, b_stride, c_stride, t_stride, first_sample, count, (hipStream_t)stream);
    return 1;
}
int nvw_set_upsampling(nvw_engine* e, const float* up_w, const float* up_b, int window, int stride) {
    if (!e->setUpsampling(up_w, up_b, window, stride)) {
        fprintf(stderr, "nvw_set_upsampling: window %d / stride %d (a multiple of the stride, at most 5 strides; nvw_set_conditioning_weights first)\n",
                window, stride);
        return 0;
    }
    return 1;
}
int nvw_set_mel(nvw_engine* e, const void* mel, int precision, long long b_stride, long long c_stride, long long f_stride, int frames) {
    const int stride = e->upsamplingStride();
    if (stride <= 0 || !wn::is_device_ptr(mel) || (precision != 32 && precision != 16) || frames <= 0 || (long long)frames * stride > e->maxSamples()) {
        fprintf(stderr, "nvw_set_mel: refused (nvw_set_upsampling first; device memory; 16- or 32-bit floats; frames * stride <= the engine's %d samples)\n",
                e->maxSamples());
        return 0;
    }
    e->setMel(mel, precision, b_stride, c_stride, f_stride, frames);
    return 1;
}
int nvw_upsample_features(nvw_engine* e, int first_sample, int count, void* stream) {
    if (e->upsamplingStride() <= 0 || e->melSamples() <= 0) {
        fprintf(stderr, "nvw_upsample_features: refused (nvw_set_upsampling and nvw_set_mel first)\n");
        return 0;
    }
    if (first_sample < 0 || count <= 0 || (long long)first_sample + count > e->melSamples()) {
        fprintf(stderr, "nvw_upsample_features: samples [%d, %lld) outside the %d the mel frames upsample to\n", first_sample,
                (long long)first_sample + count, e->melSamples());
        return 0;
    }
    e->upsampleFeatures(first_sample, count, (hipStream_t)stream);
    return 1;
}
int nvw_get_features(nvw_engine* e, void* dst, int first_sample, int count) {
    if (!e->hasFeatureBuffer() || dst == NULL || first_sample < 0 || count <= 0 || (long long)first_sample + count > e->maxSamples()) {
        fprintf(stderr, "nvw_get_features: refused (no features packed or upsampled by this engine yet, or samples [%d, %lld) outside its %d)\n",
                first_sample, (long long)first_sample + count, e->maxSamples());
        return 0;
    }
    e->getFeatures(dst, first_sample, count);
    return 1;
}
int nvw_generate_stream(nvw_engine* e, int num_samples_per_chunk, nvw_consume_fn consume, void* user, int num_samples, int batch_size, int* yOut,
                        void* stream) {
    if (e->upsamplingStride() <= 0 || e->melSamples() <= 0) {
        fprintf(stderr, "nvw_generate_stream: refused (nvw_set_upsampling and nvw_set_mel first)\n");
        return 0;
    }
    if (num_samples_per_chunk <= 0 || num_samples <= 0 || num_samples > e->melSamples() || num_samples > e->maxSamples()) {
        fprintf(stderr, "nvw_generate_stream: %d samples in chunks of %d: the mel frames upsample to %d, the engine holds %d\n", num_samples,
                num_samples_per_chunk, e->melSamples(), e->maxSamples());
        return 0;
    }
    if (batch_size <= 0 || batch_size > e->maxBatch()) {
        fprintf(stderr, "nvw_generate_stream: batch %d outside 1..%d\n", batch_size, e->maxBatch());
        return 0;
    }
    return e->run_stream(num_samples_per_chunk, consume, user, num_samples, batch_size, yOut, (hipStream_t)stream) ? 1 : 0;
}
int nvw_set_features(nvw_engine* e, const void* x, int precision, long long b_stride, long long c_stride, long long t_stride,
                     int num_samples) {
    if (!featArgsOk(e, "nvw_set_features", x, 0, num_samples) || (precision != 32 && precision != 16)) return 0;
    e->setFeatures(x, precision, b_stride, c_stride, t_stride, num_samples);
    return 1;
}
void nvw_set_selectors(nvw_engine* e, float* sel, int num_samples) { e->setSelectors(sel, num_samples); }
unsigned nvw_chain_status(nvw_engine* e) { return e->chainStatus(); }
unsigned nvw_chain_fallbacks(nvw_engine* e) { return e->chainFallbacks(); }
unsigned nvw_chain_last_timeout(nvw_engine* e) { return e->chainLastTimeout(); }
void nvw_set_chain_timeout_ms(nvw_engine* e, double ms) { e->setChainTimeoutMs(ms); }
void nvw_set_clock_probe(nvw_engine* e, int on) { e->setClockProbe(on != 0); }
void nvw_set_ring_in_lds(nvw_engine* e, int mode) { e->setRingInLds(mode); }
double nvw_last_launch_clock_ghz(nvw_engine* e) { return e->lastLaunchClockGHz(); }
int nvw_run_range(nvw_engine* e, int init_sample, int count, int num_samples, int batch_size, void* stream) {
    return e->run_range(init_sample, count, num_samples, batch_size, (hipStream_t)stream) ? 1 : 0;
}
void nvw_reset_history(nvw_engine* e, void* stream) { e->resetHistory((hipStream_t)stream); }
void nvw_set_selector_seed(nvw_engine* e, unsigned long long seed) { e->setSelectorSeed(seed); }
void nvw_set_audio_out(nvw_engine* e, short* pcmOut) { e->setAudioOut(pcmOut, 0); }
void nvw_set_audio_out_n(nvw_engine* e, short* pcmOut, size_t elems) { e->setAudioOut(pcmOut, elems); }
void nvw_kernel_info(nvw_engine* e, int batch_size, int dump_activations, char* buf, int buf_size) {
    e->kernelInfo(batch_size, dump_activations != 0, buf, buf_size);
}

int nvw_run(nvw_engine* e, int num_samples, int batch_size, int* yOut, int bspb, int dump, void* stream) {
    return e->run(num_samples, batch_size, yOut, bspb, dump != 0, (hipStream_t)stream) ? 1 : 0;
}
int nvw_run_partial(nvw_engine* e, int init_sample, int num_samples, int batch_size, int* yOut, int bspb, int dump,
                    void* stream) {
    return e->run_partial(init_sample, num_samples, batch_size, yOut, bspb, dump != 0, (hipStream_t)stream) ? 1 : 0;
}
int nvw_run_chunks(nvw_engine* e, int chunk, nvw_consume_fn consume, void* user, int num_samples, int batch_size,
                   int* yOut, int bspb, int dump, void* stream) {
    return e->run_chunks(chunk, consume, user, num_samples, batch_size, yOut, bspb, dump != 0, (hipStream_t)stream) ? 1
                                                                                                                   : 0;
}

void nvw_get_xt_out(nvw_engine* e, int layer, float* d) { e->getXtOut(layer, d); }
void nvw_get_skip_out(nvw_engine* e, int layer, float* d) { e->getSkipOut(layer, d); }
void nvw_get_zs(nvw_engine* e, float* d) { e->getZs(d); }
void nvw_get_za(nvw_engine* e, float* d) { e->getZa(d); }
void nvw_get_p(nvw_engine* e, float* d) { e->getP(d); }
void nvw_get_y_out(nvw_engine* e, int* yOut, int offset, int size, void* stream) {
    e->getYOut(yOut, offset, size, (hipStream_t)stream);
}

int nvw_slots_begin(nvw_engine* e, int window) {
    if (e->conditioningChannels() <= 0) {
        fprintf(stderr, "nvw_slots_begin: call nvw_set_conditioning_weights first\n");
        return 0;
    }
    if (e->slots().begin(window)) return 1;
    fprintf(stderr, "nvw_slots_begin: window %d is not a positive multiple of the largest dilation\n", window);
    return 0;
}
int nvw_slot_start(nvw_engine* e, int slot, const void* x, int precision, long long c_stride, long long t_stride, int length,
                   unsigned uid) {
    if (e->slots().start(slot, x, precision, c_stride, t_stride, length, uid)) return 1;
    fprintf(stderr, "nvw_slot_start: refused (nvw_slots_begin first; slot %d of %d; device features of 16 or 32 bits; strides %lld, %lld "
            "and length %d positive)\n", slot, e->maxBatch(), c_stride, t_stride, length);
    return 0;
}
int nvw_slot_stop(nvw_engine* e, int slot) {
    if (e->slots().stop(slot)) return 1;
    fprintf(stderr, "nvw_slot_stop: refused (nvw_slots_begin first; slot %d of %d)\n", slot, e->maxBatch());
    return 0;
}
int nvw_slots_step(nvw_engine* e, int count, int* yOut, short* pcm, void* stream) {
    return e->slots().step(count, yOut, pcm, (hipStream_t)stream) ? 1 : 0;
}
void nvw_slots_end(nvw_engine* e) { e->slots().end(); }
int nvw_slot_start_mel(nvw_engine* e, int slot, const void* mel, int precision, long long c_stride, long long f_stride, int frames,
                       int final, unsigned uid) {
    if (e->slots().startMel(slot, mel, precision, c_stride, f_stride, frames, final, uid)) return 1;
    fprintf(stderr, "nvw_slot_start_mel: refused (nvw_slots_begin and nvw_set_upsampling first; slot %d of %d; device frames of 16 or 32 "
            "bits; strides %lld, %lld positive; frames %d >= 0, > 0 when final)\n", slot, e->maxBatch(), c_stride, f_stride, frames);
    return 0;
}
int nvw_slot_mel_frames(nvw_engine* e, int slot, int frames, int final) {
    if (e->slots().melFrames(slot, frames, final)) return 1;
    fprintf(stderr, "nvw_slot_mel_frames: refused (slot %d of %d: not a running mel column, already final, or %d frames is fewer than "
            "before)\n", slot, e->maxBatch(), frames);
    return 0;
}
int nvw_slots_headroom(nvw_engine* e) { return e->slots().headroom(); }
int nvw_slots_get_features(nvw_engine* e, void* dst, long long first_sample, int count) {
    if (e->slots().getFeatures(dst, first_sample, count)) return 1;
    fprintf(stderr, "nvw_slots_get_features: refused (samples [%lld, %lld) are not among the last window of samples generated)\n",
            first_sample, first_sample + count);
    return 0;
}
size_t nvw_slot_state_bytes(nvw_engine* e) { return e->slots().stateBytes(); }
int nvw_slot_move(nvw_engine* e, int from, int to) {
    if (e->slots().move(from, to)) return 1;
    fprintf(stderr, "nvw_slot_move: refused (nvw_slots_begin first; %d -> %d of %d columns: a running column without a pending start, "
// ... 218 lines not shown
```

### nv_wavenet_amd/csrc/wn_kernels.hpp

```cpp
#pragma once

#include <hip/hip_runtime.h>
#include <utility>
#include <stdint.h>

#include <type_traits>

#include "wn_experiments.hpp"

namespace wn {

#define WN_DEV __device__ __forceinline__

typedef _Float16 half8 __attribute__((ext_vector_type(8)));
typedef _Float16 half4 __attribute__((ext_vector_type(4)));
typedef float floatx4 __attribute__((ext_vector_type(4)));
typedef unsigned int uintx4 __attribute__((ext_vector_type(4)));
typedef unsigned int uintx2 __attribute__((ext_vector_type(2)));

template <bool F16> struct Prec;
template <> struct Prec<true> {
    using elem = _Float16;
    using frag = half8;
    using quad = half4;
// ... 47 lines not shown
                         P_RES = P_COND + FW_COND, P_PREV = P_RES + FW_RES;
    static constexpr int FW_ZS = ATW * KF_S, FW_ZA = ATW * KF_A;
    static constexpr int FHW = FW_ZS + FW_ZA;
    static constexpr int PF = pick_pf(FLW, KFC > 0 ? WN_PFMAX_FEAT : WN_PFMAX);
    static_assert(FLW % PF == 0 && PF <= FW_ZS, "prefetch ring must divide the layer stream");
    static constexpr int HR = !F16 ? 0
                              : BT == 1 ? (FW_ZA * 4 <= WN_HEADREGS ? FW_ZA : 0)
                              : BT == 2 ? (FW_ZA * 4 <= WN_HEADREGS2 ? FW_ZA : 0)
                              : BT == 3 ? (FW_ZA * 4 <= WN_HEADREGS3 ? FW_ZA : 0)
                                        : (FW_ZA * 4 <= WN_HEADREGS4 ? FW_ZA : 0);
    static constexpr int HS = FHW - HR;
    static constexpr bool HEADRES = HS == 0;
    static constexpr int PAD1 = (PF - FW_ZS % PF) % PF, PAD2 = (PF - FW_ZA % PF) % PF;
    static constexpr int O_ZS = 0, O_ZA = FW_ZS + PAD1;
    static constexpr int FHWP = O_ZA + FW_ZA + PAD2;
    static constexpr int HSP = HS == 0 ? 0 : (HS == FW_ZS ? FW_ZS + PAD1 : FHWP);
    static_assert(HS == 0 || HS == FW_ZS || HS == FHW, "the streamed part of the head is nothing, zs, or all of it");
    __host__ __device__ static constexpr int headFrag(int q) { return q < FW_ZS ? q : q + PAD1; }
    static constexpr int FRAG_ELEMS = 64 * EPL;
    static constexpr int BIAS_L = 3 * R + S;
    static constexpr int COND_FR = 2 * HTW / TPF;
    static constexpr int LPU = 4 * NW;
    static constexpr int RPL = A / LPU;
    static_assert(RPL % 4 == 0, "A too small for the softmax lane split");
    static constexpr int XBUF = BT * KF_R * 1024;
    static constexpr int HBUF = XBUF;
    static constexpr int SKBUF = BT * KF_S * 1024;
    static constexpr int ZSBUF = BT * KF_A * 1024;
    static constexpr int LROW = A + 4;
    static constexpr int LGT = (BT >= 4 && WN_SOFTMAX_2PASS) ? 2 : BT;
    static_assert(BT % LGT == 0, "the softmax passes take whole groups of tiles");
    static constexpr int LGBUF = LGT * 16 * LROW * 4;
    static constexpr int YBUF = align16(BT * 16 * 4);
    static constexpr int XPBUF = XBUF;
    static constexpr int XPW = (KF_R + NW - 1) / NW;
    static constexpr bool ALIAS_LG = ZSBUF + LGBUF > 100 * 1024 || BT >= 3;
    static constexpr bool ZA_B_FROM_LDS = KF_A * BT * 4 > WN_ZA_B_REGS;
    static constexpr int HEADIMG = ALIAS_LG ? (ZSBUF > LGBUF ? ZSBUF : LGBUF) : ZSBUF + LGBUF;
    static constexpr bool OVERLAY = XBUF + HBUF + XPBUF <= (ALIAS_LG ? HEADIMG : LGBUF);
    static constexpr int OFF_SK = OVERLAY ? 0 : XBUF + HBUF, OFF_ZS = OFF_SK + SKBUF;
    static constexpr int OFF_LG = ALIAS_LG ? OFF_ZS : OFF_ZS + ZSBUF;
    static constexpr int OFF_Y = OFF_ZS + HEADIMG;
    static constexpr int OFF_X = OVERLAY ? OFF_LG : 0, OFF_H = OFF_X + XBUF, OFF_XP = OVERLAY ? OFF_H + HBUF : OFF_Y + YBUF;
    static constexpr int OFF_BIAS = OVERLAY ? OFF_Y + YBUF : OFF_XP + XPBUF;
    static constexpr int LDS_FIXED = XBUF + HBUF + SKBUF + HEADIMG + YBUF + XPBUF;
    static constexpr int BIAS_LN = 3 * R;
    __host__ __device__ static constexpr int biasFloats(int L, bool dump) { return (dump ? L * BIAS_L : L * BIAS_LN + S) + 2 * A; }
    __host__ __device__ static constexpr size_t ldsBytes(int L, int embTables, bool dump = true) {
        return (size_t)LDS_FIXED + (size_t)biasFloats(L, dump) * sizeof(float) + (size_t)embTables * A * R * sizeof(typename P::elem);
    }
    static constexpr int RING_SLOT = BT * KF_R * 1024;
    static constexpr int RING_INPLACE = OVERLAY ? 3 : 0;
    static_assert(XBUF == RING_SLOT && HBUF == RING_SLOT && XPBUF == RING_SLOT, "a vacated exchange image is one ring slot");
    static_assert(OFF_BIAS + RING_INPLACE * RING_SLOT == LDS_FIXED, "the in-place slots are what LDS_FIXED counts behind the tables");
    __host__ __device__ static constexpr int ringSlotOffset(int slot, int tailBase) { return tailBase + (slot - RING_INPLACE) * RING_SLOT; }
    __host__ __device__ static constexpr int ringTailSlots(int slots) { return slots > RING_INPLACE ? slots - RING_INPLACE : 0; }
    __host__ __device__ static constexpr int ldsRingSlots(int L, int maxDilation, int D) {
        int n = 0, d = 1;
        for (int l = 0; l < L; l++) {
            if (d <= D) n += d;
            d <<= 1;
            if (d > maxDilation) d = 1;
        }
        return n;
    }
    __host__ __device__ static size_t headOffsetFrags(int L) { return (size_t)L * FLW; }
    __host__ __device__ static size_t waveStreamFrags(int L) { return (size_t)L * FLW + FHWP; }
};

struct Dil {
    int d, off, lds;
};
WN_DEV Dil dil_first() { return Dil{1, 0, 0}; }
WN_DEV Dil dil_next(Dil s, int maxDilation, bool wrapToFirst, int ldsD = 0) {
    Dil n;
    n.off = s.off + s.d;
    n.lds = s.lds + (s.d <= ldsD ? s.d : 0);
    n.d = s.d << 1;
    if (n.d > maxDilation) n.d = 1;
    if (wrapToFirst) n = dil_first();
    return n;
}

struct Params {
    const void* wblob;
    const float* bias;
    const void* embPrev;
    const void* embCur;
    const void* cond;
    const void* condRaw;
    int condRawKind;
    const void* feat;
    const unsigned* gate;
    const float* sel;
    void* ring;
    int maxDilation;
    int* yInPrev;
    int* yInCur;
    int* yOut;
    float* xtOut;
    float* skipOut;
    float* zs;
    float* za;
    float* p;
    int numLayers;
    int batch;
    int maxBatch;
    int numSamples;
    int condSamples;
    int initSample;
    int count;
    int ringSlots;
    int ldsRingD;
    int tiles;
    int tileBase;
    int tanhEmbed;
    int dump;
    int embLds;
    int useRng;
    unsigned rngKey0, rngKey1;
    unsigned long long* clk;
    Dil dil[kMaxLayers + 2];
    const float* softScale;
    int forced;
};


WN_DEV float fast_exp(float x) { return __builtin_amdgcn_exp2f(x * 1.44269504088896340736f); }
WN_DEV float fast_rcp(float x) { return __builtin_amdgcn_rcpf(x); }

WN_DEV float philox_selector(unsigned k0, unsigned k1, unsigned t, unsigned b) {
    unsigned c0 = t, c1 = b, c2 = 0u, c3 = 0u;
#pragma unroll
    for (int r = 0; r < 10; r++) {
        if (r) {
            k0 += 0x9E3779B9u;
            k1 += 0xBB67AE85u;
        }
        const unsigned h0 = __umulhi(0xD2511F53u, c0), l0 = 0xD2511F53u * c0;
        const unsigned h1 = __umulhi(0xCD9E8D57u, c2), l1 = 0xCD9E8D57u * c2;
        const unsigned n0 = h1 ^ c1 ^ k0, n2 = h0 ^ c3 ^ k1;
        c0 = n0;
        c1 = l1;
        c2 = n2;
        c3 = l0;
    }
    return (float)(c0 >> 8) * (1.0f / 16777216.0f);
}

WN_DEV float sigmoid_f(float x) { return fast_rcp(1.0f + fast_exp(-x)); }

WN_DEV float tanh_fast(float x) {
    float e = fast_exp(2.0f * x);
    return 1.0f - 2.0f * fast_rcp(e + 1.0f);
}
WN_DEV float tanh_acc(float x) {
    float a = __builtin_fabsf(x);
    float x2 = x * x;
    float pz = -0.00886323552990220f;
    pz = __builtin_fmaf(pz, x2, 0.0218694885361552f);
    pz = __builtin_fmaf(pz, x2, -0.0539682539682540f);
    pz = __builtin_fmaf(pz, x2, 0.133333333333333f);
    pz = __builtin_fmaf(pz, x2, -0.333333333333333f);
    float small = __builtin_fmaf(x * x2, pz, x);
    float e = fast_exp(2.0f * a);
    float big = 1.0f - 2.0f * fast_rcp(e + 1.0f);
// ... 319 lines not shown
        }
        if (LPU >= 16) {
            up = dpp_f<0x118>(incl);
            if (sq >= 8) incl += up;
        }
    }
    total = group_reduce_f<LPU>(incl, [](float a, float b) { return __builtin_fmaxf(a, b); });
    const float target = sel * total;
    float cum = incl - lsum;
    int first = 0;
#pragma unroll
    for (int i = 0; i < RPL; i++) {
        cum += e[i];
        first += (cum <= target) ? 1 : 0;
    }
    int pick = first < RPL ? sq * RPL + first : 0x7fffffff;
    pick = group_min_i<LPU>(pick);
    if (pick >= A) pick = 128;
    return pick;
}

WN_DEV unsigned scale_pair_f32(float a, float b, float sc) {
    unsigned d;
    asm("v_fma_mixlo_f16 %0, %1, %2, 0" : "=v"(d) : "v"(a), "s"(sc));
    asm("v_fma_mixhi_f16 %0, %1, %2, 0" : "+v"(d) : "v"(b), "s"(sc));
    return d;
}
WN_DEV unsigned scale_pair_f16(unsigned h2, float sc) {
    unsigned d;
    asm("v_fma_mixlo_f16 %0, %1, %2, 0 op_sel_hi:[1,0,0]" : "=v"(d) : "v"(h2), "s"(sc));
    asm("v_fma_mixhi_f16 %0, %1, %2, 0 op_sel:[1,0,0] op_sel_hi:[1,0,0]" : "+v"(d) : "v"(h2), "s"(sc));
    return d;
}
template <bool F16, int RAW, int CR> WN_DEV typename Prec<F16>::frag cond_frag(const typename Prec<F16>::frag (&c)[CR], int k) {
    if constexpr (RAW == 1 && F16) {
        const floatx4 a = __builtin_bit_cast(floatx4, c[2 * k]), b = __builtin_bit_cast(floatx4, c[2 * k + 1]);
        const float st = gate_prescale<true>(false), ss = gate_prescale<true>(true);
        return __builtin_bit_cast(half8, uintx4{scale_pair_f32(a[0], a[1], st), scale_pair_f32(a[2], a[3], st),
                                                scale_pair_f32(b[0], b[1], ss), scale_pair_f32(b[2], b[3], ss)});
    } else if constexpr (RAW == 2 && F16) {
        const uintx4 q = __builtin_bit_cast(uintx4, c[k]);
        const float st = gate_prescale<true>(false), ss = gate_prescale<true>(true);
        return __builtin_bit_cast(half8, uintx4{scale_pair_f16(q[0], st), scale_pair_f16(q[1], st), scale_pair_f16(q[2], ss),
                                                scale_pair_f16(q[3], ss)});
    } else {
        return c[k];
    }
}

WN_DEV float fma_mix_lo(unsigned h2, float acc) {
    float d;
    asm("v_fma_mix_f32 %0, %1, 1.0, %2 op_sel_hi:[1,0,0]" : "=v"(d) : "v"(h2), "v"(acc));
    return d;
}
WN_DEV float fma_mix_hi(unsigned h2, float acc) {
    float d;
    asm("v_fma_mix_f32 %0, %1, 1.0, %2 op_sel:[1,0,0] op_sel_hi:[1,0,0]" : "=v"(d) : "v"(h2), "v"(acc));
    return d;
}
template <bool F16> WN_DEV void cond_add(floatx4* a, typename Prec<F16>::frag c, const typename Prec<F16>::frag* selA) {
    if constexpr (F16) {
#if WN_COND_VALU
        (void)selA;
        const uintx4 q = __builtin_bit_cast(uintx4, c);
        a[0][0] = fma_mix_lo(q[0], a[0][0]);
        a[0][1] = fma_mix_hi(q[0], a[0][1]);
        a[0][2] = fma_mix_lo(q[1], a[0][2]);
        a[0][3] = fma_mix_hi(q[1], a[0][3]);
        a[1][0] = fma_mix_lo(q[2], a[1][0]);
        a[1][1] = fma_mix_hi(q[2], a[1][1]);
        a[1][2] = fma_mix_lo(q[3], a[1][2]);
        a[1][3] = fma_mix_hi(q[3], a[1][3]);
#else
#pragma unroll
        for (int tt = 0; tt < Prec<F16>::TPF; tt++) a[tt] = mma(selA[tt], c, a[tt]);
#endif
    } else {
        (void)selA;
#pragma unroll
        for (int e = 0; e < Prec<F16>::EPL; e++) a[e >> 2][e & 3] += (float)c[e];
    }
}

template <bool F16, int R, int S, int A, int BT, bool EMBLDS, bool DUMP = true, int RAW = 0, bool LR = false>
#ifdef WN_EXP_TWO_WG
__global__ __launch_bounds__((Cfg<F16, R, S, A, BT>::THREADS), (BT == 1 ? 2 : 1)) void wavenet_wg(const Params p) {
#else
__global__ __launch_bounds__((Cfg<F16, R, S, A, BT>::THREADS), 1) void wavenet_wg(const Params p) {
#endif
    constexpr bool FEAT = RAW == 3;
    constexpr int KFC = FEAT ? feat_kfc<F16>() : 0;
    using C = Cfg<F16, R, S, A, BT, KFC>;
    using P = Prec<F16>;
    using frag = typename P::frag;
    using quad = typename P::quad;
    using elem = typename P::elem;
    constexpr int PF = C::PF, FLW = C::FLW, FHW = C::FHW, NW = C::NW;
    constexpr int RT = C::RT, HTW = C::HTW, STW = C::STW, ATW = C::ATW;
    constexpr int KF_R = C::KF_R, KF_S = C::KF_S, KF_A = C::KF_A;

    extern __shared__ __attribute__((aligned(16))) char lds[];
    char* const xbuf = lds + C::OFF_X;
    char* const hbuf = lds + C::OFF_H;
    char* const skbuf = lds + C::OFF_SK;
    char* const zsbuf = lds + C::OFF_ZS;
    float* const lgbuf = (float*)(lds + C::OFF_LG);
    int* const ybuf = (int*)(lds + C::OFF_Y);
    char* const xpbuf = lds + C::OFF_XP;
    float* const biasLds = (float*)(lds + C::OFF_BIAS);

    static_assert(RAW == 0 || RAW == 1 || (RAW == 2 && F16) || RAW == 3, "RAW: 0 packed, 1 fp32 in place, 2 fp16 in place (fp16 engine), 3 features");
    if (p.gate != nullptr && __builtin_nontemporal_load(p.gate) == 0u) return;

    const int tid = threadIdx.x;
    const int lane = tid & 63;
    const int w = __builtin_amdgcn_readfirstlane(tid >> 6);
    const int g = lane >> 4, j = lane & 15;
    const int L = p.numLayers;
    const int tile0 = p.tileBase + blockIdx.x * BT;
    if (p.clk != nullptr && blockIdx.x == 0 && tid == 0) {
        p.clk[0] = __builtin_amdgcn_s_memtime();
        p.clk[1] = __builtin_amdgcn_s_memrealtime();
    }

    int ub[BT];
    bool uvalid[BT];
#pragma unroll
    for (int bt = 0; bt < BT; bt++) {
        const int b = (tile0 + bt) * 16 + j;
        uvalid[bt] = b < p.batch;
        ub[bt] = uvalid[bt] ? b : p.batch - 1;
    }
    const int su = tid / C::LPU, sq = tid % C::LPU;

    constexpr int BLS = DUMP ? C::BIAS_L : C::BIAS_LN;
    if constexpr (DUMP) {
        const int nb = L * C::BIAS_L + 2 * A;
        for (int i = tid; i < nb; i += C::THREADS) biasLds[i] = p.bias[i];
        __syncthreads();
        for (int s0 = tid; s0 < S; s0 += C::THREADS) {
            float run = biasLds[3 * R + s0];
            for (int l = 1; l < L; l++) {
                run += biasLds[l * C::BIAS_L + 3 * R + s0];
                biasLds[l * C::BIAS_L + 3 * R + s0] = run;
            }
        }
    } else {
        for (int i = tid; i < L * C::BIAS_LN; i += C::THREADS) biasLds[i] = p.bias[(i / C::BIAS_LN) * C::BIAS_L + i % C::BIAS_LN];
        for (int i = tid; i < 2 * A; i += C::THREADS) biasLds[L * C::BIAS_LN + S + i] = p.bias[L * C::BIAS_L + i];
        for (int s0 = tid; s0 < S; s0 += C::THREADS) {
            float run = p.bias[3 * R + s0];
            for (int l = 1; l < L; l++) run += p.bias[l * C::BIAS_L + 3 * R + s0];
            biasLds[L * C::BIAS_LN + s0] = run;
        }
    }
    const float* const skipBiasSum = DUMP ? biasLds + (L - 1) * C::BIAS_L + 3 * R : biasLds + L * C::BIAS_LN;
    const float* const headBias = biasLds + (C::biasFloats(L, DUMP) - 2 * A);

    const unsigned laneOff = (unsigned)lane * 16u;
    const char* const wbase = (const char*)p.wblob + (size_t)w * C::waveStreamFrags(L) * 1024;
    const char* const whead = wbase + C::headOffsetFrags(L) * 1024;
    const elem* embPrev = (const elem*)p.embPrev;
    const elem* embCur = (const elem*)p.embCur;
    if constexpr (EMBLDS) {
        elem* const embLds = (elem*)(biasLds + C::biasFloats(L, DUMP));
        const floatx4* s0 = (const floatx4*)p.embCur;
        const floatx4* s1 = (const floatx4*)p.embPrev;
        constexpr int CH = (int)(A * R * sizeof(elem) / 16);
        for (int i = tid; i < CH; i += C::THREADS) {
            ((floatx4*)embLds)[i] = s0[i];
            if (p.embLds > 1) ((floatx4*)embLds)[CH + i] = s1[i];
        }
        embCur = embLds;
        if (p.embLds > 1) embPrev = embLds + A * R;
        __syncthreads();
    }

    int yPrev[BT], yCur[BT];
    floatx4 ep[BT][HTW];
#pragma unroll
    for (int bt = 0; bt < BT; bt++) {
        yPrev[bt] = p.yInPrev[ub[bt]];
        yCur[bt] = p.yInCur[ub[bt]];
#pragma unroll
        for (int i = 0; i < HTW; i++)
            ep[bt][i] = quad_to_f32(*(const quad*)(embPrev + (size_t)yPrev[bt] * R + (w + NW * i) * 16 + g * 4));
    }

    constexpr bool ws_pin = F16 && !(RAW == 1 && BT == 2);
    WStream<F16, PF, ws_pin> ws;
    const rsrc_t rsW = make_rsrc(wbase);
#pragma unroll
    for (int i = 0; i < PF; i++) ws.buf[i] = buf_load<frag, WN_W_AUX>(rsW, laneOff + (unsigned)(i & 3) * 1024u, (unsigned)(i & ~3) * 1024u);

    constexpr int HR = C::HR, HS = C::HS;
    frag hw[HR ? HR : 1];
    if constexpr (HR > 0) {
#pragma unroll
        for (int i = 0; i < HR; i++) hw[i] = *(const frag*)(whead + (size_t)C::headFrag(HS + i) * 1024 + laneOff);
    }

    constexpr int XPW = C::XPW;
    frag xpA[BT][XPW], xpB[BT][XPW];
    constexpr int CR = (RAW == 1 && F16) ? 2 * C::COND_FR : C::COND_FR;
    frag cdA[BT][CR], cdB[BT][CR];
    constexpr int KFCR = FEAT ? KFC : 1;
    frag cfCur[BT][KFCR], cfNext[BT][KFCR];
    const size_t featStride = (size_t)p.tiles * KFC * 1024;
    const char* const featMine = (const char*)p.feat + (size_t)tile0 * KFC * 1024;
    auto load_feat = [&](int tn, frag (&dst)[BT][KFCR]) {
        const int tc = tn < p.condSamples ? tn : p.condSamples - 1;
        const rsrc_t rsF = make_rsrc(featMine + (size_t)tc * featStride);
#pragma unroll
        for (int bt = 0; bt < BT; bt++)
#pragma unroll
            for (int k = 0; k < KFC; k++)
                dst[bt][k] = buf_load<frag, WN_FEAT_AUX>(rsF, laneOff + (unsigned)(k & 3) * 1024u, (unsigned)((bt * KFC + (k & ~3)) * 1024));
    };
    const size_t condStride = (size_t)p.tiles * NW * C::COND_FR * 1024;
    const char* const condMine = (const char*)p.cond + ((size_t)tile0 * NW + w) * C::COND_FR * 1024;
    const size_t ringTile = (size_t)p.ringSlots * KF_R * 1024;
    char* const ringMine = (char*)p.ring + (size_t)tile0 * ringTile;
    const rsrc_t rsRing = make_rsrc(ringMine);
    const unsigned ringTileB = (unsigned)ringTile;
    const int ldsD = LR ? p.ldsRingD : 0;
    char* const ringLds = lds + C::ringSlotOffset(0, (int)C::ldsBytes(L, EMBLDS ? p.embLds : 0, DUMP));
    const char* condNext = condMine + (size_t)p.initSample * L * condStride;
    constexpr unsigned RAWE = RAW == 2 ? 2u : 4u;
    const size_t rawRow = (size_t)p.maxBatch * (2 * R) * RAWE;
    unsigned rawOff[BT];
#pragma unroll
    for (int bt = 0; bt < BT; bt++) rawOff[bt] = ((unsigned)ub[bt] * (unsigned)(2 * R) + (unsigned)g * 4u) * RAWE;
    auto prefetch = [&](int tn, int ln, Dil dl, frag (&xd)[BT][XPW], frag (&cdd)[BT][CR]) {
        if (ln >= L) { ln -= L; tn += 1; }
        const unsigned slot = (unsigned)(dl.off + (tn & (dl.d - 1)));
        const unsigned rp0 = slot * (unsigned)(KF_R * 1024);
        const rsrc_t rsCond = make_rsrc(condNext);
        condNext += condStride;
        if (dl.d > ldsD) {
#pragma unroll
            for (int i = 0; i < XPW; i++) {
                const int k = w + NW * i;
                if (k < KF_R) {
#pragma unroll
                    for (int bt = 0; bt < BT; bt++)
                        xd[bt][i] = buf_load<frag, WN_RING_LD_AUX>(rsRing, laneOff, rp0 + (unsigned)bt * ringTileB + (unsigned)k * 1024u);
                }
            }
        }
#pragma unroll
        for (int bt = 0; bt < BT; bt++) {
            if constexpr (FEAT) {
            } else if constexpr (RAW != 0) {
                const int tc = tn < p.condSamples ? tn : p.condSamples - 1;
                const rsrc_t rsRaw = make_rsrc((const char*)p.condRaw + ((size_t)tc * L + ln) * rawRow);
                auto slotOff = [&](int it) { return (unsigned)((w + NW * (it >> 1) + (it & 1) * RT) * 16) * RAWE; };
                if constexpr (RAW == 1) {
#pragma unroll
                    for (int it = 0; it < 2 * HTW; it++) cdd[bt][it] = buf_load<frag, WN_RAW_AUX>(rsRaw, rawOff[bt], slotOff(it));
                } else {
#pragma unroll
                    for (int k = 0; k < HTW; k++) {
                        const uintx2 qa = __builtin_amdgcn_raw_buffer_load_b64(rsRaw, rawOff[bt], slotOff(2 * k), WN_RAW_AUX);
                        const uintx2 qb = __builtin_amdgcn_raw_buffer_load_b64(rsRaw, rawOff[bt], slotOff(2 * k + 1), WN_RAW_AUX);
                        cdd[bt][k] = __builtin_bit_cast(frag, uintx4{qa[0], qa[1], qb[0], qb[1]});
                    }
                }
            } else {
#pragma unroll
                for (int k = 0; k < C::COND_FR; k++)
                    cdd[bt][k] = buf_load<frag, WN_COND_AUX>(rsCond, laneOff + (unsigned)(k & 3) * 1024u,
                                                   (unsigned)((bt * NW * C::COND_FR + (k & ~3)) * 1024));
            }
        }
    };
    auto ring_lds_copy = [&](auto TOLDS) {
        constexpr bool toLds = decltype(TOLDS)::value;
        if (ldsD <= 0) return;
        Dil dl = dil_first();
        for (int l = 0; l < L; l++) {
            if (dl.d <= ldsD) {
                const int rows = dl.d * BT * KF_R;
                for (int r = w; r < rows; r += NW) {
                    const int sl = r / (BT * KF_R), bt = (r / KF_R) % BT, k = r % KF_R;
                    const unsigned hb = (unsigned)(dl.off + sl) * (unsigned)(KF_R * 1024) + (unsigned)bt * ringTileB + (unsigned)k * 1024u;
                    char* const lp = ringLds + (size_t)(dl.lds + sl) * C::RING_SLOT + ((bt * KF_R + k) * 64 + lane) * 16;
                    if constexpr (toLds) *(frag*)lp = buf_load<frag, WN_RING_LD_AUX>(rsRing, laneOff, hb);
                    else buf_store<frag, WN_RING_ST_AUX>(rsRing, laneOff, hb, *(const frag*)lp);
                }
            }
            dl = dil_next(dl, p.maxDilation, false, ldsD);
        }
    };
    ring_lds_copy(std::true_type{});
    prefetch(p.initSample, 0, p.dil[0], xpA, cdA);
    prefetch(p.initSample, 1, p.dil[1], xpB, cdB);
    auto publish_xp = [&](const frag (&xpN)[BT][XPW], const Dil dN) {
        if (dN.d <= ldsD) return;
#pragma unroll
        for (int i = 0; i < XPW; i++) {
            const int k = w + NW * i;
            if (k < KF_R) {
#pragma unroll
                for (int bt = 0; bt < BT; bt++) *(frag*)(xpbuf + ((bt * KF_R + k) * 64 + lane) * 16) = xpN[bt][i];
            }
        }
    };
    auto tap_image = [&](const Dil dN, int tn) -> const char* {
        return dN.d <= ldsD ? ringLds + (size_t)(dN.lds + (tn & (dN.d - 1))) * C::RING_SLOT : xpbuf;
    };
    publish_xp(xpA, p.dil[0]);

    __syncthreads();

#ifdef WN_TIMING
    unsigned long long tacc[12] = {0};
    unsigned long long tmark = 0;
#define WN_TMARK(i)                                                        \
    {                                                                      \
        unsigned long long _n = __builtin_amdgcn_s_memtime();              \
        asm volatile("s_waitcnt lgkmcnt(0)" ::: "memory");                 \
        tacc[i] += _n - tmark;                                             \
        tmark = _n;                                                        \
    }
#else
#define WN_TMARK(i)
#endif
    frag selA[P::TPF];
#pragma unroll
    for (int tt = 0; tt < P::TPF; tt++)
#pragma unroll
        for (int e = 0; e < P::EPL; e++)
            selA[tt][e] = (elem)(((e >> 2) == tt && g * 4 + (e & 3) == j) ? 1.0f : 0.0f);
    floatx4 acc[BT][2 * HTW];
    {
        frag xp[BT][KF_R];
#pragma unroll
        for (int bt = 0; bt < BT; bt++) {
            lds_get_frags<F16, KF_R>(tap_image(p.dil[0], p.initSample) + bt * KF_R * 1024, lane, xp[bt]);
#pragma unroll
            for (int i = 0; i < HTW; i++) {
                acc[bt][2 * i] = *(const floatx4*)(biasLds + (w + NW * i) * 16 + g * 4);
                acc[bt][2 * i + 1] = *(const floatx4*)(biasLds + (w + NW * i + RT) * 16 + g * 4);
            }
        }
        if constexpr (FEAT) {
            load_feat(p.initSample, cfNext);
#pragma unroll
            for (int bt = 0; bt < BT; bt++)
#pragma unroll
                for (int k = 0; k < KFC; k++) cfCur[bt][k] = agpr_operand<F16>(cfNext[bt][k]);
            gemm_direct<F16, BT, 2 * HTW, KFC>(wbase + C::streamPos(0, C::O_COND, L) * 1024, laneOff, acc, cfCur);
            load_feat(p.initSample + 1, cfNext);
#pragma unroll
            for (int bt = 0; bt < BT; bt++)
#pragma unroll
                for (int k = 0; k < KFC; k++) asm volatile("" ::"v"(cfNext[bt][k]));
        } else {
#pragma unroll
            for (int bt = 0; bt < BT; bt++)
#pragma unroll
                for (int k = 0; k < C::COND_FR; k++) cond_add<F16>(&acc[bt][k * P::TPF], cond_frag<F16, RAW>(cdA[bt], k), selA);
        }
        gemm_direct<F16, BT, 2 * HTW, KF_R>(wbase + C::streamPos(0, C::O_PREV, L) * 1024, laneOff, acc, xp);
    }
    float sscale[FEAT ? BT : 1];
    if constexpr (FEAT) {
#pragma unroll
        for (int bt = 0; bt < BT; bt++) {
            int sb = (tile0 + bt) * 16 + su;
            sb = sb < p.batch ? sb : p.batch - 1;
            sscale[bt] = p.softScale != nullptr ? p.softScale[sb] : kLog2e;
        }
    }
    const int tEnd = p.initSample + p.count;
    for (int t = p.initSample; t < tEnd; t++) {
        const bool dumpNow = DUMP && p.dump && (t == tEnd - 1);

        float selv[BT];
        if (!p.useRng) {
#pragma unroll
            for (int bt = 0; bt < BT; bt++) {
                int sb = (tile0 + bt) * 16 + su;
                sb = sb < p.batch ? sb : p.batch - 1;
                selv[bt] = p.sel[(size_t)t * p.maxBatch + sb];
            }
        }

        WN_TMARK(11)
        floatx4 x[BT][HTW];
#pragma unroll
        for (int bt = 0; bt < BT; bt++) {
#pragma unroll
            for (int i = 0; i < HTW; i++) {
                const int tile = w + NW * i;
                floatx4 ec = quad_to_f32(*(const quad*)(embCur + (size_t)yCur[bt] * R + tile * 16 + g * 4));
                floatx4 v = ep[bt][i] + ec;
                if (p.tanhEmbed) {
#pragma unroll
                    for (int r = 0; r < 4; r++) v[r] = tanh_t<F16>(v[r]);
                }
                x[bt][i] = v;
                lds_put_tile<F16>(xbuf + bt * KF_R * 1024, tile, lane, v);
            }
#pragma unroll
            for (int i = 0; i < HTW; i++)
                ep[bt][i] = quad_to_f32(*(const quad*)(embPrev + (size_t)yCur[bt] * R + (w + NW * i) * 16 + g * 4));
        }
        wg_barrier();
        WN_TMARK(0)

        floatx4 skip[BT][STW];
#pragma unroll
        for (int bt = 0; bt < BT; bt++)
#pragma unroll
            for (int i = 0; i < STW; i++) skip[bt][i] = floatx4{0.f, 0.f, 0.f, 0.f};

        frag hb[BT][KF_R];
        frag xb[BT][KF_R];
#pragma unroll
        for (int bt = 0; bt < BT; bt++) lds_get_frags<F16, KF_R>(xbuf + bt * KF_R * 1024, lane, xb[bt]);
        auto layer = [&](auto withSkip, const int l, const Dil dl, const Dil dN, const Dil dl2, frag (&xpC)[BT][XPW],
                         frag (&cdC)[BT][CR], const frag (&xpN)[BT][XPW], const frag (&cdN)[BT][CR]) {
            constexpr bool SKIP = decltype(withSkip)::value;
            constexpr int PB = SKIP ? 0 : FLW;
            const int wl = SKIP ? (l - 1) * FLW : 0;
            const float* bl = biasLds + l * BLS;
            const int lN = l + 1 < L ? l + 1 : 0;
            const float* blN = biasLds + lN * BLS;
            const int d = dl.d;

            WN_TMARK(1)
            gemm_b<F16, PF, 0, BT, 2 * HTW, KF_R>(ws, rsW, SKIP ? C::P_CUR : C::P_CUR0 - PB, wl, 0, laneOff, acc, xb);
            const bool ringInLds = d <= ldsD;
            frag xkeep[BT][XPW];
            if (!ringInLds) {
                const unsigned rp = (unsigned)(dl.off + (t & (d - 1))) * (unsigned)(KF_R * 1024);
#pragma unroll
                for (int k = 0; k < KF_R; k++)
                    if (k % NW == w) {
#pragma unroll
                        for (int bt = 0; bt < BT; bt++)
                            buf_store<frag, WN_RING_ST_AUX>(rsRing, laneOff + (unsigned)(k & 3) * 1024u,
                                               rp + (unsigned)bt * ringTileB + (unsigned)(k & ~3) * 1024u, xb[bt][k]);
                    }
            } else {
#pragma unroll
                for (int k = 0; k < KF_R; k++)
                    if (k % NW == w) {
#pragma unroll
                        for (int bt = 0; bt < BT; bt++) xkeep[bt][k / NW] = xb[bt][k];
                    }
            }
            if constexpr (!SKIP) prefetch(t, l + 2, dl2, xpC, cdC);
            __builtin_amdgcn_sched_barrier(0);
            WN_TMARK(2)

            floatx4 accN[FEAT ? BT : 1][2 * HTW];
            if constexpr (FEAT) {
#pragma unroll
                for (int bt = 0; bt < BT; bt++)
#pragma unroll
                    for (int i = 0; i < HTW; i++) {
                        accN[bt][2 * i] = *(const floatx4*)(blN + (w + NW * i) * 16 + g * 4);
                        accN[bt][2 * i + 1] = *(const floatx4*)(blN + (w + NW * i + RT) * 16 + g * 4);
                    }
            }
            if constexpr (FEAT) {
                constexpr int NS = BT * HTW * 2 * 5;
                constexpr int NFS = SKIP ? STW * KF_R : 0, NFC = C::FW_COND;
                constexpr int NM = (NFS + NFC) * BT;
                constexpr int G0S = STW >= 4 ? 4 : STW, G0C = 2 * HTW >= 4 ? 4 : 2 * HTW;
                constexpr bool EARLY = PF > 1;
                floatx2 ea, eb, ra, rb, hp;
                floatx4 hv;
                auto stage = [&](auto SI) {
                    constexpr int s = decltype(SI)::value, pr = s / 5, st = s % 5;
                    constexpr int bt = pr / (2 * HTW), i = (pr / 2) % HTW, r = (pr & 1) * 2;
                    gate_stage<F16, st>(acc[bt][2 * i][r], acc[bt][2 * i][r + 1], acc[bt][2 * i + 1][r], acc[bt][2 * i + 1][r + 1],
                                        ea, eb, ra, rb, hp);
                    if constexpr (st == 4) {
                        hv[r] = hp[0];
                        hv[r + 1] = hp[1];
                        if constexpr (r == 2) lds_put_tile<F16>(hbuf + bt * KF_R * 1024, w + NW * i, lane, hv);
                    }
                    __builtin_amdgcn_sched_barrier(0);
                };
                static_for<NFS + NFC>([&](auto FI) {
                    constexpr int fi = decltype(FI)::value;
                    constexpr bool isSkip = fi < NFS;
                    constexpr int q = isSkip ? fi : fi - NFS, G0 = isSkip ? G0S : G0C, KFq = isSkip ? KF_R : KFC;
                    constexpr int kf = (q / G0) % KFq, mt = (q / (G0 * KFq)) * G0 + q % G0;
                    constexpr int pos = isSkip ? C::P_SKIP + q : C::P_COND - PB + q;
                    constexpr int posPrev = (fi - 1 < NFS) ? C::P_SKIP + fi - 1 : C::P_COND - PB + fi - 1 - NFS;
                    frag a[1];
                    take_group<F16, PF, ws_pin, 1>(ws, pos, a);
                    if constexpr (EARLY && fi > 0) refill_group<F16, PF, 0, ws_pin, 1>(ws, rsW, posPrev, wl, 0, laneOff);
                    static_for<BT>([&](auto BI) {
                        constexpr int bt = decltype(BI)::value, m = fi * BT + bt;
                        if constexpr (isSkip) skip[bt][mt] = mma(a[0], hb[bt][kf], skip[bt][mt]);
                        else accN[bt][mt] = mma(a[0], cfCur[bt][kf], accN[bt][mt]);
                        __builtin_amdgcn_sched_barrier(0);
                        static_for_range<m * NS / NM, (m + 1) * NS / NM>(stage);
                    });
                    if constexpr (!EARLY || fi == NFS + NFC - 1) refill_group<F16, PF, 0, ws_pin, 1>(ws, rsW, pos, wl, 0, laneOff);
                    if constexpr (SKIP && fi == (NFS + NFC) * WN_REQ_AT_FEAT / 8) {
                        prefetch(t, l + 2, dl2, xpC, cdC);
                        __builtin_amdgcn_sched_barrier(0);
                    }
                });
                if (l == L - 2) {
                    asm volatile("");
#pragma unroll
                    for (int bt = 0; bt < BT; bt++)
#pragma unroll
                        for (int k = 0; k < KFC; k++) cfCur[bt][k] = agpr_operand<F16>(cfNext[bt][k]);
                }
                if constexpr (SKIP) {
                    if (dumpNow) {
                        const float* bp = biasLds + (l - 1) * C::BIAS_L + 3 * R;
#pragma unroll
                        for (int bt = 0; bt < BT; bt++) {
                            if (!uvalid[bt]) continue;
#pragma unroll
                            for (int i = 0; i < STW; i++)
                                *(floatx4*)(p.skipOut + ((size_t)(l - 1) * p.maxBatch + ub[bt]) * S + (w + NW * i) * 16 + g * 4) =
                                    skip[bt][i] + *(const floatx4*)(bp + (w + NW * i) * 16 + g * 4);
                        }
                    }
                }
            } else {
                constexpr int NS = BT * HTW * 2 * 5;
                constexpr int NM = SKIP ? STW * KF_R * BT : 0;
                floatx2 ea, eb, ra, rb, hp;
                floatx4 hv;
                auto stage = [&](auto SI) {
                    constexpr int s = decltype(SI)::value, pr = s / 5, st = s % 5;
                    constexpr int bt = pr / (2 * HTW), i = (pr / 2) % HTW, r = (pr & 1) * 2;
                    gate_stage<F16, st>(acc[bt][2 * i][r], acc[bt][2 * i][r + 1], acc[bt][2 * i + 1][r], acc[bt][2 * i + 1][r + 1],
                                        ea, eb, ra, rb, hp);
                    if constexpr (st == 4) {
                        hv[r] = hp[0];
                        hv[r + 1] = hp[1];
                        if constexpr (r == 2) lds_put_tile<F16>(hbuf + bt * KF_R * 1024, w + NW * i, lane, hv);
                    }
                    __builtin_amdgcn_sched_barrier(0);
                };
                if constexpr (SKIP) {
                    constexpr int G0 = STW >= 4 ? 4 : STW, G = take_g(G0, PF);
                    static_for<STW * KF_R / G>([&](auto GI) {
                        constexpr int gi = decltype(GI)::value, q = gi * G;
                        constexpr int kf = (q / G0) % KF_R, mg = q / (G0 * KF_R), mi0 = q % G0;
                        frag a[G];
                        take_group<F16, PF, ws_pin, G>(ws, C::P_SKIP + gi * G, a);
                        constexpr bool EARLY = PF > G;
                        if constexpr (EARLY && gi > 0) refill_group<F16, PF, 0, ws_pin, G>(ws, rsW, C::P_SKIP + (gi - 1) * G, wl, 0, laneOff);
                        static_for<G * BT>([&](auto MI) {
                            constexpr int mi = decltype(MI)::value / BT, bt = decltype(MI)::value % BT;
                            constexpr int mt = mg * G0 + mi0 + mi, m = (q + mi) * BT + bt;
                            skip[bt][mt] = mma(a[mi], hb[bt][kf], skip[bt][mt]);
                            __builtin_amdgcn_sched_barrier(0);
                            static_for_range<m * NS / NM, (m + 1) * NS / NM>(stage);
                        });
                        if constexpr (!EARLY || gi == STW * KF_R / G - 1) refill_group<F16, PF, 0, ws_pin, G>(ws, rsW, C::P_SKIP + gi * G, wl, 0, laneOff);
                        if constexpr (gi == (STW * KF_R / G) * WN_REQ_AT / 8) {
                            prefetch(t, l + 2, dl2, xpC, cdC);
                            __builtin_amdgcn_sched_barrier(0);
                        }
                    });
                    if (dumpNow) {
                        const float* bp = biasLds + (l - 1) * C::BIAS_L + 3 * R;
#pragma unroll
                        for (int bt = 0; bt < BT; bt++) {
                            if (!uvalid[bt]) continue;
#pragma unroll
                            for (int i = 0; i < STW; i++)
                                *(floatx4*)(p.skipOut + ((size_t)(l - 1) * p.maxBatch + ub[bt]) * S + (w + NW * i) * 16 + g * 4) =
                                    skip[bt][i] + *(const floatx4*)(bp + (w + NW * i) * 16 + g * 4);
                        }
                    }
                } else {
                    static_for<NS>(stage);
                }
            }
            WN_TMARK(3)
            wg_barrier();
            WN_TMARK(4)
#pragma unroll
            for (int bt = 0; bt < BT; bt++) lds_get_frags<F16, KF_R>(hbuf + bt * KF_R * 1024, lane, hb[bt]);
            if (ringInLds) {
                char* const sl = ringLds + (size_t)(dl.lds + (t & (d - 1))) * C::RING_SLOT;
#pragma unroll
                for (int i = 0; i < XPW; i++) {
                    const int k = w + NW * i;
                    if (k < KF_R) {
#pragma unroll
                        for (int bt = 0; bt < BT; bt++) *(frag*)(sl + ((bt * KF_R + k) * 64 + lane) * 16) = xkeep[bt][i];
                    }
                }
            }

            floatx4 xa[BT][HTW];
#pragma unroll
            for (int bt = 0; bt < BT; bt++)
#pragma unroll
                for (int i = 0; i < HTW; i++)
                    xa[bt][i] = *(const floatx4*)(bl + 2 * R + (w + NW * i) * 16 + g * 4) + x[bt][i];
#pragma unroll
            for (int bt = 0; bt < BT; bt++)
#pragma unroll
                for (int i = 0; i < HTW; i++) {
                    if constexpr (FEAT) {
                        acc[bt][2 * i] = accN[bt][2 * i];
                        acc[bt][2 * i + 1] = accN[bt][2 * i + 1];
                    } else {
                        acc[bt][2 * i] = *(const floatx4*)(blN + (w + NW * i) * 16 + g * 4);
                        acc[bt][2 * i + 1] = *(const floatx4*)(blN + (w + NW * i + RT) * 16 + g * 4);
                    }
                }

            gemm_b<F16, PF, 0, BT, HTW, KF_R>(ws, rsW, C::P_RES - PB, wl, 0, laneOff, xa, hb);
#pragma unroll
            for (int bt = 0; bt < BT; bt++)
#pragma unroll
                for (int i = 0; i < HTW; i++) {
                    x[bt][i] = xa[bt][i];
                    lds_put_tile<F16>(xbuf + bt * KF_R * 1024, w + NW * i, lane, xa[bt][i]);
                }
            publish_xp(xpN, dN);
            __builtin_amdgcn_sched_barrier(0);
            WN_TMARK(5)
            if constexpr (FEAT) {
            } else {
#pragma unroll
                for (int bt = 0; bt < BT; bt++)
#pragma unroll
                    for (int k = 0; k < C::COND_FR; k++) cond_add<F16>(&acc[bt][k * P::TPF], cond_frag<F16, RAW>(cdN[bt], k), selA);
            }
            if (dumpNow) {
#pragma unroll
                for (int bt = 0; bt < BT; bt++) {
                    if (!uvalid[bt]) continue;
#pragma unroll
                    for (int i = 0; i < HTW; i++)
                        *(floatx4*)(p.xtOut + ((size_t)l * p.maxBatch + ub[bt]) * R + (w + NW * i) * 16 + g * 4) = x[bt][i];
                }
            }
            __builtin_amdgcn_sched_barrier(0);
            WN_TMARK(6)
            wg_barrier();
            WN_TMARK(7)
            frag xp[BT][KF_R];
            const char* const tapImg = tap_image(dN, l + 1 < L ? t : t + 1);
#pragma unroll
            for (int bt = 0; bt < BT; bt++) lds_get_frags<F16, KF_R>(tapImg + bt * KF_R * 1024, lane, xp[bt]);
#pragma unroll
            for (int bt = 0; bt < BT; bt++) lds_get_frags<F16, KF_R>(xbuf + bt * KF_R * 1024, lane, xb[bt]);
            __builtin_amdgcn_sched_barrier(0);
            gemm_b<F16, PF, 0, BT, 2 * HTW, KF_R>(ws, rsW, C::P_PREV - PB, wl, 0, laneOff, acc, xp);
        };
        {
            Dil da = dil_first(), db = dil_next(da, p.maxDilation, L == 1, ldsD), dc = dil_next(db, p.maxDilation, L == 2, ldsD);
            auto adv = [&](int l) { da = db; db = dc; dc = dil_next(dc, p.maxDilation, l + 3 == L, ldsD); };
            layer(std::false_type{}, 0, da, db, dc, xpA, cdA, xpB, cdB);
            adv(0);
            int l = 1;
            for (; l + 1 < L; l += 2) {
                layer(std::true_type{}, l, da, db, dc, xpB, cdB, xpA, cdA);
                adv(l);
                layer(std::true_type{}, l + 1, da, db, dc, xpA, cdA, xpB, cdB);
                adv(l + 1);
            }
            if (l < L) layer(std::true_type{}, l, da, db, dc, xpB, cdB, xpA, cdA);
            if (L & 1) {
#pragma unroll
                for (int bt = 0; bt < BT; bt++) {
#pragma unroll
                    for (int i = 0; i < XPW; i++) {
                        const frag tmp = xpA[bt][i];
                        xpA[bt][i] = xpB[bt][i];
                        xpB[bt][i] = tmp;
                    }
#pragma unroll
                    for (int k = 0; k < CR; k++) {
                        const frag tmp = cdA[bt][k];
                        cdA[bt][k] = cdB[bt][k];
                        cdB[bt][k] = tmp;
                    }
                }
            }
        }
        gemm_b<F16, PF, 0, BT, STW, KF_R>(ws, rsW, C::P_CUR, (L - 1) * FLW, 0, laneOff, skip, hb);

#pragma unroll
        for (int bt = 0; bt < BT; bt++)
#pragma unroll
            for (int i = 0; i < STW; i++) {
                floatx4 v = skip[bt][i] + *(const floatx4*)(skipBiasSum + (w + NW * i) * 16 + g * 4);
#pragma unroll
                for (int r = 0; r < 4; r++) v[r] = __builtin_fmaxf(v[r], 0.f);
                lds_put_tile<F16>(skbuf + bt * KF_S * 1024, w + NW * i, lane, v);
                if (dumpNow && uvalid[bt])
                    *(floatx4*)(p.skipOut + ((size_t)(L - 1) * p.maxBatch + ub[bt]) * S + (w + NW * i) * 16 + g * 4) = v;
            }
        wg_barrier();
        floatx4 zs[BT][ATW];
        if constexpr (HS != 0 && KF_S * BT * 4 > WN_ZS_B_REGS) {
#pragma unroll
            for (int bt = 0; bt < BT; bt++)
#pragma unroll
                for (int i = 0; i < ATW; i++) zs[bt][i] = *(const floatx4*)(headBias + (w + NW * i) * 16 + g * 4);
            gemm_ldsb_b<F16, PF, C::HSP, BT, ATW, KF_S>(ws, rsW, C::O_ZS, L * FLW, 0, laneOff, zs, skbuf, lane);
            skip_frags<F16, PF, C::HSP, ws_pin, C::PAD1>(ws, rsW, C::FW_ZS, L * FLW, 0, laneOff);
        } else {
            frag sb[BT][KF_S];
#pragma unroll
            for (int bt = 0; bt < BT; bt++) {
                lds_get_frags<F16, KF_S>(skbuf + bt * KF_S * 1024, lane, sb[bt]);
#pragma unroll
                for (int i = 0; i < ATW; i++) zs[bt][i] = *(const floatx4*)(headBias + (w + NW * i) * 16 + g * 4);
            }
            if constexpr (HS == 0) gemm_res<F16, BT, ATW, KF_S>(hw, 0, zs, sb);
            else {
                gemm_b<F16, PF, C::HSP, BT, ATW, KF_S>(ws, rsW, C::O_ZS, L * FLW, 0, laneOff, zs, sb);
                skip_frags<F16, PF, C::HSP, ws_pin, C::PAD1>(ws, rsW, C::FW_ZS, L * FLW, 0, laneOff);
            }
        }
#pragma unroll
        for (int bt = 0; bt < BT; bt++)
#pragma unroll
            for (int i = 0; i < ATW; i++) {
#pragma unroll
                for (int r = 0; r < 4; r++) zs[bt][i][r] = __builtin_fmaxf(zs[bt][i][r], 0.f);
                lds_put_tile<F16>(zsbuf + bt * KF_A * 1024, w + NW * i, lane, zs[bt][i]);
                if (dumpNow && uvalid[bt])
                    *(floatx4*)(p.zs + (size_t)ub[bt] * A + (w + NW * i) * 16 + g * 4) = zs[bt][i];
            }
        wg_barrier();
        floatx4 za[BT][ATW];
        {
#pragma unroll
            for (int bt = 0; bt < BT; bt++)
#pragma unroll
                for (int i = 0; i < ATW; i++)
                    za[bt][i] = *(const floatx4*)(headBias + A + (w + NW * i) * 16 + g * 4);
            auto draw_selectors = [&]() {
                if (!p.useRng) return;
                if constexpr (C::LPU == 16 && BT > 1) {
                    const int q = sq < BT ? sq : 0;
                    int sb = (tile0 + q) * 16 + su;
                    sb = sb < p.batch ? sb : p.batch - 1;
                    const float mine = philox_selector(p.rngKey0, p.rngKey1, (unsigned)t, (unsigned)sb);
                    selv[0] = dpp_f<0x150>(mine);
                    if constexpr (BT > 1) selv[1] = dpp_f<0x151>(mine);
                    if constexpr (BT > 2) selv[2] = dpp_f<0x152>(mine);
                    if constexpr (BT > 3) selv[3] = dpp_f<0x153>(mine);
// ... 20 lines not shown
            }
        }
        if constexpr (C::ALIAS_LG) wg_barrier();
        constexpr int LGT = C::LGT;
        auto put_logits = [&](auto PASS) {
            constexpr int pass = decltype(PASS)::value;
#pragma unroll
            for (int bl = 0; bl < LGT; bl++)
#pragma unroll
                for (int i = 0; i < ATW; i++) {
                    const int bt = pass * LGT + bl;
                    *(floatx4*)(lgbuf + (bl * 16 + j) * C::LROW + (w + NW * i) * 16 + g * 4) = za[bt][i];
                    if (dumpNow && uvalid[bt])
                        *(floatx4*)(p.za + (size_t)ub[bt] * A + (w + NW * i) * 16 + g * 4) = za[bt][i];
                }
        };
        put_logits(std::integral_constant<int, 0>{});
        WN_TMARK(8)
        if constexpr (HS == FHW) {
            skip_frags<F16, PF, C::HSP, ws_pin, C::PAD2>(ws, rsW, C::O_ZA + C::FW_ZA, L * FLW, 0, laneOff);
        }
        if constexpr (FEAT) load_feat(t + 2, cfNext);
        wg_barrier();
        WN_TMARK(9)

        static_for<BT / LGT>([&](auto PASS) {
            constexpr int pass = decltype(PASS)::value;
            if constexpr (pass > 0) {
                wg_barrier();
                put_logits(PASS);
                wg_barrier();
            }
#pragma unroll
            for (int bl = 0; bl < LGT; bl++) {
                const int bt = pass * LGT + bl;
                float e[C::RPL];
                float total;
                const float* lrow = lgbuf + (bl * 16 + su) * C::LROW + sq * C::RPL;
                int pick;
                if constexpr (FEAT) {
                    pick = softmax_pick<A, C::LPU, C::RPL>(lrow, sq, lane, selv[bt], e, total, sscale[bt]);
                    if (p.forced) pick = selv[bt] <= -1.0f ? (int)(-selv[bt]) - 1 : pick;
                } else pick = softmax_pick<A, C::LPU, C::RPL>(lrow, sq, lane, selv[bt], e, total);
                const int sb = (tile0 + bt) * 16 + su;
                if (sq == 0) {
                    ybuf[bt * 16 + su] = pick;
                    if (sb < p.batch) p.yOut[(size_t)sb * p.numSamples + t] = pick;
                }
                if (dumpNow && sb < p.batch) {
                    const float inv = 1.0f / total;
#pragma unroll
                    for (int i = 0; i < C::RPL / 4; i++)
                        *(floatx4*)(p.p + (size_t)sb * A + sq * C::RPL + i * 4) =
                            floatx4{e[i * 4] * inv, e[i * 4 + 1] * inv, e[i * 4 + 2] * inv, e[i * 4 + 3] * inv};
                }
            }
        });
        wg_barrier();
#pragma unroll
        for (int bt = 0; bt < BT; bt++) {
            yPrev[bt] = yCur[bt];
            yCur[bt] = ybuf[bt * 16 + j];
        }
        WN_TMARK(10)
    }
#ifdef WN_TIMING
    if (tid == 0 && blockIdx.x == 0)
        for (int i = 0; i < 12; i++) p.p[i] = (float)tacc[i];
#endif

    ring_lds_copy(std::false_type{});
    if (w == 0 && g == 0) {
#pragma unroll
        for (int bt = 0; bt < BT; bt++)
            if (uvalid[bt]) {
                p.yInPrev[ub[bt]] = yPrev[bt];
                p.yInCur[ub[bt]] = yCur[bt];
            }
    }
    if (p.clk != nullptr && blockIdx.x == 0 && tid == 0) {
        p.clk[2] = __builtin_amdgcn_s_memtime();
        p.clk[3] = __builtin_amdgcn_s_memrealtime();
    }
}

static __global__ void mulaw_pcm_kernel(const int* __restrict__ yOut, short* __restrict__ pcm,
                                        const short* __restrict__ table, int batch, int numSamples, int first,
                                        int count) {
    const size_t n = (size_t)batch * count;
    for (size_t i = blockIdx.x * (size_t)blockDim.x + threadIdx.x; i < n; i += (size_t)gridDim.x * blockDim.x) {
        const size_t at = (i / count) * numSamples + first + (i % count);
        pcm[at] = table[yOut[at]];
    }
}


template <bool F16>
WN_DEV void pack_weight_elem(typename Prec<F16>::elem* __restrict__ dst, const float* __restrict__ src, int M, int K,
                             int NW, size_t waveStride, int gateRT, size_t idx) {
    constexpr int EPL = Prec<F16>::EPL, TPF = Prec<F16>::TPF;
    const int KF = K / (16 * TPF);
    const int tilesPerWave = M / 16 / NW;
    const size_t perWave = (size_t)tilesPerWave * KF * 64 * EPL;
    const int w = idx / perWave;
    size_t r = idx % perWave;
    const int e = r % EPL; r /= EPL;
    const int lane = r % 64; r /= 64;
    const int G = tilesPerWave >= 4 ? 4 : tilesPerWave;
    const int mi = r % G;
    const int kf = (r / G) % KF;
    const int it = (r / (G * KF)) * G + mi;
    int tile;
    if (gateRT > 0) tile = w + NW * (it >> 1) + (it & 1) * gateRT;
    else tile = w + NW * it;
    const int i = lane & 15, g = lane >> 4;
    const int m = tile * 16 + i;
    const int k = (kf * TPF + (e >> 2)) * 16 + g * 4 + (e & 3);
    float v = src[(size_t)m + (size_t)k * M];
    if (gateRT > 0) v *= gate_prescale<F16>(m >= M / 2);
    dst[(size_t)w * waveStride + (idx % perWave)] = (typename Prec<F16>::elem)v;
}
template <bool F16>
__global__ void pack_weight_kernel(typename Prec<F16>::elem* __restrict__ dst, const float* __restrict__ src, int M,
                                   int K, int NW, size_t waveStride, int gateRT) {
    const size_t n = (size_t)M * K;
    for (size_t idx = (size_t)blockIdx.x * blockDim.x + threadIdx.x; idx < n; idx += (size_t)gridDim.x * blockDim.x)
        pack_weight_elem<F16>(dst, src, M, K, NW, waveStride, gateRT, idx);
}

struct LayerSrc {
    const float *Wprev, *Wcur, *Bh, *Wres, *Bres, *Wskip, *Bskip;
};
template <bool F16>
__global__ void pack_layer_kernel(typename Prec<F16>::elem* __restrict__ layerFrags, float* __restrict__ biasL, LayerSrc s,
                                  int R, int S, int NW, size_t waveStride, int oPrev, int oCur, int oRes, int oSkip) {
    constexpr int FE = 64 * Prec<F16>::EPL;
    const size_t nGate = (size_t)2 * R * R, nRes = (size_t)R * R, nSkip = (size_t)S * R;
    const size_t nW = 2 * nGate + nRes + nSkip, n = nW + 3 * R + S;
    for (size_t idx = (size_t)blockIdx.x * blockDim.x + threadIdx.x; idx < n; idx += (size_t)gridDim.x * blockDim.x) {
        if (idx < nGate) pack_weight_elem<F16>(layerFrags + (size_t)oPrev * FE, s.Wprev, 2 * R, R, NW, waveStride, R / 16, idx);
        else if (idx < 2 * nGate) pack_weight_elem<F16>(layerFrags + (size_t)oCur * FE, s.Wcur, 2 * R, R, NW, waveStride, R / 16, idx - nGate);
        else if (idx < 2 * nGate + nRes) pack_weight_elem<F16>(layerFrags + (size_t)oRes * FE, s.Wres, R, R, NW, waveStride, 0, idx - 2 * nGate);
        else if (idx < nW) pack_weight_elem<F16>(layerFrags + (size_t)oSkip * FE, s.Wskip, S, R, NW, waveStride, 0, idx - 2 * nGate - nRes);
        else {
            const int i = (int)(idx - nW);
            if (i < 2 * R) biasL[i] = s.Bh[i] * gate_prescale<F16>(i >= R);
            else if (i < 3 * R) biasL[i] = s.Bres[i - 2 * R];
            else biasL[i] = s.Bskip[i - 3 * R];
        }
    }
}

template <bool F16>
__global__ void convert_kernel(typename Prec<F16>::elem* __restrict__ dst, const float* __restrict__ src, size_t n) {
    for (size_t i = (size_t)blockIdx.x * blockDim.x + threadIdx.x; i < n; i += (size_t)gridDim.x * blockDim.x)
        dst[i] = (typename Prec<F16>::elem)src[i];
}

template <bool F16, int R>
__global__ __launch_bounds__(256) void pack_cond_tiled_kernel(typename Prec<F16>::elem* __restrict__ dst,
                                                              const float* __restrict__ src, size_t rows, int maxBatch,
                                                              int tiles) {
    using elem = typename Prec<F16>::elem;
    using frag = typename Prec<F16>::frag;
    constexpr int EPL = Prec<F16>::EPL, TPF = Prec<F16>::TPF;
    constexpr int R2 = 2 * R, RT = R / 16, NW = RT >= 4 ? 4 : RT;
// ... 238 lines not shown
```

### nv_wavenet_amd/engine.py

```python
import ctypes as C

import numpy as np

from ._lib import lib, addr, CONSUME_FN

SLOT_PIECE = np.dtype([("slot", "<i4"), ("uid", "<u4"), ("first", "<i8"), ("n", "<i4"), ("finished", "<i4"), ("offset", "<i8")])
assert SLOT_PIECE.itemsize == 32
SLOT_SAVED = np.dtype([("slot", "<i4"), ("uid", "<u4"), ("done", "<i4"), ("mel", "<i4")])
SLOT_RESUME_REQ = np.dtype({"names": ["slot", "mel", "src", "precision", "c_stride", "t_stride", "length", "final"],
                            "formats": ["<i4", "<i4", "<u8", "<i4", "<i8", "<i8", "<i4", "<i4"],
                            "offsets": [0, 4, 8, 16, 24, 32, 40, 44], "itemsize": 48})
assert SLOT_SAVED.itemsize == 16
PREFILL_REQ = np.dtype({"names": ["y", "n", "x", "precision", "c_stride", "t_stride", "uid", "temperature"],
                        "formats": ["<u8", "<i4", "<u8", "<i4", "<i8", "<i8", "<u4", "<f4"],
                        "offsets": [0, 8, 16, 24, 32, 40, 48, 52], "itemsize": 56})
SCORE_REQ = np.dtype({"names": ["y", "n", "x", "precision", "c_stride", "t_stride", "temperature", "logp", "rows"],
                      "formats": ["<u8", "<i4", "<u8", "<i4", "<i8", "<i8", "<f4", "<u8", "<u8"],
                      "offsets": [0, 8, 16, 24, 32, 40, 48, 56, 64], "itemsize": 72})
UPSAMPLE_REQ = np.dtype({"names": ["mel", "precision", "c_stride", "f_stride", "frames", "first_sample", "count", "dst"],
                         "formats": ["<u8", "<i4", "<i8", "<i8", "<i4", "<i4", "<i4", "<u8"],
                         "offsets": [0, 8, 16, 24, 32, 36, 40, 48], "itemsize": 56})
PREFILL_MEL_REQ = np.dtype({"names": ["y", "n", "mel", "precision", "c_stride", "f_stride", "frames", "uid", "temperature"],
                            "formats": ["<u8", "<i4", "<u8", "<i4", "<i8", "<i8", "<i4", "<u4", "<f4"],
                            "offsets": [0, 8, 16, 24, 32, 40, 48, 52, 56], "itemsize": 64})
# ... 173 lines not shown
            raise ValueError("nvw_pack_features refused samples [%d, %d)" % (firstSample, firstSample + x.size(2)))

    def setConditioningFeatures(self, frags, numSamples=None):
        import torch
        assert hasattr(frags, "data_ptr") and frags.is_cuda and frags.is_contiguous()
        want = torch.float16 if self.precision == 16 else torch.float32
        assert frags.dtype == want, "an fp%d engine reads %s fragments" % (self.precision, want)
        ns = frags.size(0) if numSamples is None else int(numSamples)
        self._cond_keep = frags
        if not lib.nvw_set_conditioning_features(self._h, addr(frags), ns, frags.numel()):
            raise ValueError("the feature fragment tensor does not fit %d samples" % ns)

    def setUpsampling(self, upW, upB, stride):
        W, b = _f32(upW), _f32(upB)
        window = int(W.shape[2])
        assert tuple(W.shape[:2]) == (self.nCond, self.nCond), "upsample weight must be [n_cond][n_cond][window]"
        if not lib.nvw_set_upsampling(self._h, addr(W), addr(b), window, int(stride)):
            raise ValueError("upsampling window %d / stride %d not supported" % (window, stride))
        self.upStride = int(stride)

    def setMel(self, mel):
        bits, sb, sc, sf = self._feat_args(mel)
        assert mel.size(0) == self.maxBatch and mel.size(1) == self.nCond
        self._cond_keep = None
        if not lib.nvw_set_mel(self._h, mel.data_ptr(), bits, sb, sc, sf, mel.size(2)):
            raise ValueError("nvw_set_mel refused %s" % (tuple(mel.shape),))
        self.melFrames = mel.size(2)

    def upsampleFeatures(self, firstSample, count, stream=None):
        if not lib.nvw_upsample_features(self._h, int(firstSample), int(count), stream):
            raise ValueError("nvw_upsample_features refused samples [%d, %d)" % (firstSample, firstSample + count))

    def getFeatures(self, firstSample, count):
        import torch
        epl = 8 if self.precision == 16 else 4
        out = torch.empty(count, self.condTiles(), self.featureFragments(), 4, 16, epl, device="cuda",
                          dtype=torch.float16 if self.precision == 16 else torch.float32)
        if not lib.nvw_get_features(self._h, out.data_ptr(), int(firstSample), int(count)):
            raise ValueError("nvw_get_features refused samples [%d, %d)" % (firstSample, firstSample + count))
        return out

    def generate_stream(self, num_samples_per_chunk, consume, num_samples, batch_size, yOut=None, stream=None):
        def _cb(_ptr, init, count, _user):
            if consume is not None:
                consume(yOut, init, count)
        cb = CONSUME_FN(_cb)
        self._cb_keep = cb
        return bool(lib.nvw_generate_stream(self._h, int(num_samples_per_chunk), cb, None, int(num_samples), int(batch_size),
                                            self._yout(yOut, num_samples), stream))

    def setSelectors(self, outputSelectors, numSamples=None):
        sel = _f32(outputSelectors)
        ns = self.maxSamples if numSamples is None else int(numSamples)
        assert (sel.numel() if hasattr(sel, "numel") else sel.size) == ns * self.maxBatch
        lib.nvw_set_selectors(self._h, addr(sel), ns)

    def packConditioning(self, Lh, firstSample, count, stream=None):
        Lh = _f32(Lh)
        assert hasattr(Lh, "data_ptr") and Lh.is_cuda, "packConditioning takes device tensors"
        assert Lh.numel() == count * self.numLayers * self.maxBatch * 2 * self.R
        self._cond_keep = None
        lib.nvw_pack_conditioning(self._h, addr(Lh), int(firstSample), int(count), stream)

    def run_partial_chunk(self, init_sample, count, num_samples, batch_size, stream=None):
        return bool(lib.nvw_run_range(self._h, int(init_sample), int(count), int(num_samples), int(batch_size), stream))

    def resetHistory(self, stream=None):
        lib.nvw_reset_history(self._h, stream)

    def chainStatus(self):
        return int(lib.nvw_chain_status(self._h))

    def chainFallbacks(self):
        return int(lib.nvw_chain_fallbacks(self._h))

    def chainLastTimeout(self):
        return int(lib.nvw_chain_last_timeout(self._h))

    def setChainTimeoutMs(self, ms):
        lib.nvw_set_chain_timeout_ms(self._h, float(ms))

    def setRingInLds(self, mode=0):
        lib.nvw_set_ring_in_lds(self._h, int(mode))

    def setClockProbe(self, on=True):
        lib.nvw_set_clock_probe(self._h, 1 if on else 0)

    def lastLaunchClockGHz(self):
        return float(lib.nvw_last_launch_clock_ghz(self._h))

    def kernelInfo(self, batch_size=None, dumpActivations=False):
        import ctypes
        buf = ctypes.create_string_buffer(256)
        lib.nvw_kernel_info(self._h, self.maxBatch if batch_size is None else batch_size, 1 if dumpActivations else 0,
                            buf, 256)
        return buf.value.decode()

    def setSelectorSeed(self, seed):
        lib.nvw_set_selector_seed(self._h, int(seed) & 0xFFFFFFFFFFFFFFFF)

    def setAudioOut(self, pcmOut):
        if pcmOut is not None:
            if hasattr(pcmOut, "data_ptr"):
                import torch
                assert pcmOut.dtype == torch.int16
            else:
                assert pcmOut.dtype == np.int16 and pcmOut.flags["C_CONTIGUOUS"]
            n = pcmOut.numel() if hasattr(pcmOut, "numel") else pcmOut.size
            self._pcm_keep = pcmOut
            lib.nvw_set_audio_out_n(self._h, addr(pcmOut), n)
        else:
            self._pcm_keep = None
            lib.nvw_set_audio_out(self._h, None)

    def slotsBegin(self, window):
        if not lib.nvw_slots_begin(self._h, int(window)):
            raise ValueError("nvw_slots_begin refused window %d (conditioning weights first; a multiple of the largest dilation)" % window)
        self.slotWindow = int(window)
        self._slot_keep = {}

    def slotStart(self, slot, x, uid, length=None):
        import torch
        assert hasattr(x, "data_ptr") and x.is_cuda and x.dim() == 2, "features: a CUDA tensor [n_cond][samples]"
        bits = {torch.float32: 32, torch.float16: 16}.get(x.dtype)
        assert bits, "features must be float32 or float16"
        n = x.size(1) if length is None else int(length)
        assert x.size(0) == self.nCond and 0 < n <= x.size(1), "features [%d][>= %d] expected, got %s" % (self.nCond, n, tuple(x.shape))
        if not lib.nvw_slot_start(self._h, int(slot), x.data_ptr(), bits, x.stride(0), x.stride(1), n, int(uid) & 0xFFFFFFFF):
            raise ValueError("nvw_slot_start refused slot %d" % slot)
        self._slot_keep[int(slot)] = x

    def slotStop(self, slot):
        if not lib.nvw_slot_stop(self._h, int(slot)):
            raise ValueError("nvw_slot_stop refused slot %d" % slot)

    def slotsStep(self, count, yOut=None, pcm=None, stream=None):
        for a, name in ((yOut, "yOut"), (pcm, "pcm")):
            if a is not None:
                n = a.numel() if hasattr(a, "numel") else a.size
                assert n >= self.maxBatch * count, "%s must hold [maxBatch][count]" % name
        if yOut is not None:
            self._yout(yOut, count)
        if pcm is not None and not hasattr(pcm, "data_ptr"):
            assert pcm.dtype == np.int16 and pcm.flags["C_CONTIGUOUS"]
        return bool(lib.nvw_slots_step(self._h, int(count), addr(yOut), addr(pcm), stream))

    def slotsStepRagged(self, count, samples=None, pcm=None, stream=None):
        cap = None
        for a, dt, name in ((samples, "int32", "samples"), (pcm, "int16", "pcm")):
            if a is not None:
                assert hasattr(a, "data_ptr") and (a.is_cuda or a.is_pinned()) and a.is_contiguous() and str(a.dtype) == "torch." + dt, \
                    "%s: a contiguous CUDA or pinned %s tensor" % (name, dt)
                cap = a.numel() if cap is None else min(cap, a.numel())
        pieces = np.empty(self.maxBatch, dtype=SLOT_PIECE)
        n, ticket = C.c_int(0), C.c_ulonglong(0)
        total = lib.nvw_slots_step_ragged(self._h, int(count), addr(samples), addr(pcm), cap or 0, pieces.ctypes.data, self.maxBatch,
                                          C.byref(n), C.byref(ticket), stream)
        if total == -2:
            raise RuntimeError("nvw_slots_step_ragged: a launch of the step of %d samples failed" % count)
        if total < 0:
            raise ValueError("nvw_slots_step_ragged refused a step of %d samples into %s elements" % (count, cap))
        return int(total), pieces[:n.value], int(ticket.value)

    def slotsWait(self, ticket):
        if not lib.nvw_slots_wait(self._h, int(ticket)):
            raise ValueError("nvw_slots_wait: no ticket %d" % ticket)
# ... 412 lines not shown
```

Measured before the change: 322.7 million samples/s.

## Add compile-time dilation schedule kernel for cyclic 10-layer fp16 configs

Adds a specialized kernel variant in which the dilation cycle (dilations 1..512 repeating every 10 layers) is unrolled at compile time. Ring offsets, LDS slot indices and wrap flags become constexpr, replacing the runtime dil_next bookkeeping. LDS ring use is capped at dilation 1 or 2 for this path. It is on by default when the config matches (fp16, BT=3, maxDilation=512, layers a multiple of 10). The cost is a larger kernel body from full unrolling, with possible register pressure, and fewer ring taps held in LDS than the runtime plan might have chosen.

```diff
diff --git a/include/nv_wavenet_c.h b/include/nv_wavenet_c.h
--- a/include/nv_wavenet_c.h
+++ b/include/nv_wavenet_c.h
@@ -62,6 +62,7 @@
 void nvw_set_chain_timeout_ms(nvw_engine* e, double ms);
 void nvw_set_clock_probe(nvw_engine* e, int on);
 void nvw_set_ring_in_lds(nvw_engine* e, int mode);
+void nvw_set_compiled_schedule(nvw_engine* e, int mode);
 double nvw_last_launch_clock_ghz(nvw_engine* e);
 int nvw_run_range(nvw_engine* e, int init_sample, int count, int num_samples, int batch_size, void* stream);
 void nvw_reset_history(nvw_engine* e, void* stream);
diff --git a/nv_wavenet_amd/_lib.py b/nv_wavenet_amd/_lib.py
--- a/nv_wavenet_amd/_lib.py
+++ b/nv_wavenet_amd/_lib.py
@@ -56,6 +56,7 @@
     "nvw_set_chain_timeout_ms": (None, [C.c_void_p, C.c_double]),
     "nvw_set_clock_probe": (None, [C.c_void_p, C.c_int]),
     "nvw_set_ring_in_lds": (None, [C.c_void_p, C.c_int]),
+    "nvw_set_compiled_schedule": (None, [C.c_void_p, C.c_int]),
     "nvw_last_launch_clock_ghz": (C.c_double, [C.c_void_p]),
     "nvw_run_range": (C.c_int, [C.c_void_p, C.c_int, C.c_int, C.c_int, C.c_int, C.c_void_p]),
     "nvw_reset_history": (None, [C.c_void_p, C.c_void_p]),
diff --git a/nv_wavenet_amd/csrc/engine_base.hpp b/nv_wavenet_amd/csrc/engine_base.hpp
--- a/nv_wavenet_amd/csrc/engine_base.hpp
+++ b/nv_wavenet_amd/csrc/engine_base.hpp
@@ -40,6 +40,7 @@
     virtual void setChainTimeoutMs(double) = 0;
     virtual void setClockProbe(bool) = 0;
     virtual void setRingInLds(int) = 0;
+    virtual void setCompiledSchedule(int) = 0;
     virtual double lastLaunchClockGHz() = 0;
     virtual int precisionBits() = 0;
     virtual int maxSamples() = 0;
@@ -205,6 +206,7 @@
     void setChainTimeoutMs(double ms) override { eng.setChainTimeoutMs(ms); }
     void setClockProbe(bool on) override { eng.setClockProbe(on); }
     void setRingInLds(int mode) override { eng.setRingInLds(mode); }
+    void setCompiledSchedule(int mode) override { eng.setCompiledSchedule(mode); }
     double lastLaunchClockGHz() override { return eng.lastLaunchClockGHz(); }
     int precisionBits() override { return std::is_same<Td, float>::value ? 32 : 16; }
     int maxSamples() override { return cap; }
diff --git a/nv_wavenet_amd/csrc/nv_wavenet.hpp b/nv_wavenet_amd/csrc/nv_wavenet.hpp
--- a/nv_wavenet_amd/csrc/nv_wavenet.hpp
+++ b/nv_wavenet_amd/csrc/nv_wavenet.hpp
@@ -65,6 +65,7 @@
     int m_num_samples_per_chunk;
     int m_ringSlots;
     int m_ringDirtyTiles;
+    int m_schedMode;
     int m_ringLdsMode;
     int m_lastStride;
 
@@ -215,6 +216,23 @@
         p = q;
         return bytes;
     }
+    static constexpr int kCycle = 10;
+    static constexpr bool schedBuilt(int bt, bool dump, int raw) { return F16 && WG3 && bt == 3 && !dump && raw == 0; }
+    int compiledSchedule(int bt, bool dump, int raw, int ringD) const {
+        if (!schedBuilt(bt, dump, raw) || m_schedMode < 0) return 0;
+        if (m_maxDilation != (1 << (kCycle - 1)) || m_numLayers % kCycle != 0 || ringD < 1) return 0;
+        return ringD >= 2 ? 2 : 1;
+    }
+    void capLdsRing(wn::Params& p, int D) const {
+        p.ldsRingD = D;
+        int slot = 0;
+        for (int l = 0; l < m_numLayers; l++) {
+            p.dil[l].lds = slot;
+            if (p.dil[l].d <= D) slot += p.dil[l].d;
+        }
+        p.dil[m_numLayers] = p.dil[0];
+        p.dil[m_numLayers + 1] = p.dil[1];
+    }
     template <int BT, bool EMB, bool DUMP, int RAW> bool launchK(wn::Params& p, int tiles, int nEmb, hipStream_t stream) {
         using CB = wn::Cfg<F16, R, S, A, BT>;
         const int grid = (tiles + BT - 1) / BT;
@@ -222,6 +240,15 @@
         const size_t need = ldsNeed<BT>(m_numLayers, nEmb, DUMP);
         if constexpr (lrBuilt(DUMP, RAW)) {
             const size_t ringBytes = ringPlan<BT>(p, need, DUMP, RAW);
+            if constexpr (schedBuilt(BT, DUMP, RAW)) {
+                const int ld = compiledSchedule(BT, DUMP, RAW, p.ldsRingD);
+                if (ld > 0) {
+                    capLdsRing(p, 1 << (ld - 1));
+                    if (ld == 2) hipLaunchKernelGGL((wn::wavenet_wg_cs<F16, R, S, A, BT, EMB, kCycle, 2>), dim3(grid), dim3(CB::THREADS), need + ringBytes, stream, p);
+                    else hipLaunchKernelGGL((wn::wavenet_wg_cs<F16, R, S, A, BT, EMB, kCycle, 1>), dim3(grid), dim3(CB::THREADS), need + ringBytes, stream, p);
+                    return hipGetLastError() == hipSuccess;
+                }
+            }
             if (p.ldsRingD > 0) {
                 hipLaunchKernelGGL((wn::wavenet_wg<F16, R, S, A, BT, EMB, DUMP, RAW, true>), dim3(grid), dim3(CB::THREADS), need + ringBytes, stream, p);
                 return hipGetLastError() == hipSuccess;
@@ -272,6 +299,12 @@
             if constexpr (lrBuilt(DUMP, RAW))
                 gpuErrChk(hipFuncSetAttribute((const void*)wn::wavenet_wg<F16, R, S, A, BT, EMB, DUMP, RAW, true>,
                                               hipFuncAttributeMaxDynamicSharedMemorySize, (int)kLdsMax));
+            if constexpr (schedBuilt(BT, DUMP, RAW)) {
+                gpuErrChk(hipFuncSetAttribute((const void*)wn::wavenet_wg_cs<F16, R, S, A, BT, EMB, kCycle, 1>,
+                                              hipFuncAttributeMaxDynamicSharedMemorySize, (int)kLdsMax));
+                gpuErrChk(hipFuncSetAttribute((const void*)wn::wavenet_wg_cs<F16, R, S, A, BT, EMB, kCycle, 2>,
+                                              hipFuncAttributeMaxDynamicSharedMemorySize, (int)kLdsMax));
+            }
         }
     }
     template <int BT, bool DUMP> void allowLdsD() {
@@ -406,6 +439,7 @@
         assert(numLayers >= 2 && batchSize > 0 && numSamples > 0 && maxDilation > 0);
         m_ringDirtyTiles = 0;
         m_ringLdsMode = 0;
+        m_schedMode = 0;
         assert(numLayers <= wn::kMaxLayers);
         {
             int dev = 0;
@@ -576,6 +610,7 @@
         return (double)(c[2] - c[0]) / (double)(c[3] - c[1]) * (double)wallKHz * 1e-6;
     }
     void setRingInLds(int mode) { m_ringLdsMode = mode < 0 ? -1 : 0; }
+    void setCompiledSchedule(int mode) { m_schedMode = mode < 0 ? -1 : 0; }
     void setChainTimeoutMs(double ms) { m_chainTimeoutTicks = (long long)(ms * 1e5); }
 
     virtual void setEmbeddings(float* embedPrev, float* embedCur) {
@@ -958,8 +993,10 @@
             lds += rb;
             ringD = q.ldsRingD;
         }
-        char ring[48] = "";
-        if (ringD > 0) snprintf(ring, sizeof(ring), " ring_in_lds=d<=%d", ringD);
+        const int ld = compiledSchedule(bt, dump, raw, ringD);
+        if (ld > 0) ringD = 1 << (ld - 1);
+        char ring[64] = "";
+        if (ringD > 0) snprintf(ring, sizeof(ring), " ring_in_lds=d<=%d%s", ringD, ld > 0 ? " sched=cycle10" : "");
         snprintf(buf, n, "wn::wavenet_wg<%s,%d,%d,%d,BT=%d,EMBLDS=%d,DUMP=%d,RAW=%d%s> tiles/wg=%d wgs=%d lds=%zu%s",
                  F16 ? "fp16" : "fp32", R, S, A, bt, nEmb, dump ? 1 : 0, raw, ringD > 0 ? ",LR=1" : "", bt, (tiles + bt - 1) / bt, lds, ring);
     }
diff --git a/nv_wavenet_amd/csrc/wavenet_capi.hip b/nv_wavenet_amd/csrc/wavenet_capi.hip
--- a/nv_wavenet_amd/csrc/wavenet_capi.hip
+++ b/nv_wavenet_amd/csrc/wavenet_capi.hip
@@ -225,6 +225,7 @@
 void nvw_set_chain_timeout_ms(nvw_engine* e, double ms) { e->setChainTimeoutMs(ms); }
 void nvw_set_clock_probe(nvw_engine* e, int on) { e->setClockProbe(on != 0); }
 void nvw_set_ring_in_lds(nvw_engine* e, int mode) { e->setRingInLds(mode); }
+void nvw_set_compiled_schedule(nvw_engine* e, int mode) { e->setCompiledSchedule(mode); }
 double nvw_last_launch_clock_ghz(nvw_engine* e) { return e->lastLaunchClockGHz(); }
 int nvw_run_range(nvw_engine* e, int init_sample, int count, int num_samples, int batch_size, void* stream) {
     return e->run_range(init_sample, count, num_samples, batch_size, (hipStream_t)stream) ? 1 : 0;
diff --git a/nv_wavenet_amd/csrc/wn_kernels.hpp b/nv_wavenet_amd/csrc/wn_kernels.hpp
--- a/nv_wavenet_amd/csrc/wn_kernels.hpp
+++ b/nv_wavenet_amd/csrc/wn_kernels.hpp
@@ -153,6 +153,12 @@
     return n;
 }
 
+template <int I, int LD> struct DilC {
+    static constexpr int d = 1 << I;
+    int off, lds;
+    WN_DEV DilC(int cycleOff, int cycleLds) : off(cycleOff + (1 << I) - 1), lds(cycleLds + (1 << (I < LD ? I : LD)) - 1) {}
+};
+
 struct Params {
     const void* wblob;
     const float* bias;
@@ -638,12 +644,8 @@
     }
 }
 
-template <bool F16, int R, int S, int A, int BT, bool EMBLDS, bool DUMP = true, int RAW = 0, bool LR = false>
-#ifdef WN_EXP_TWO_WG
-__global__ __launch_bounds__((Cfg<F16, R, S, A, BT>::THREADS), (BT == 1 ? 2 : 1)) void wavenet_wg(const Params p) {
-#else
-__global__ __launch_bounds__((Cfg<F16, R, S, A, BT>::THREADS), 1) void wavenet_wg(const Params p) {
-#endif
+template <bool F16, int R, int S, int A, int BT, bool EMBLDS, bool DUMP, int RAW, bool LR, int CYC, int LD>
+WN_DEV void wavenet_wg_body(const Params& p) {
     constexpr bool FEAT = RAW == 3;
     constexpr int KFC = FEAT ? feat_kfc<F16>() : 0;
     using C = Cfg<F16, R, S, A, BT, KFC>;
@@ -666,6 +668,7 @@
     float* const biasLds = (float*)(lds + C::OFF_BIAS);
 
     static_assert(RAW == 0 || RAW == 1 || (RAW == 2 && F16) || RAW == 3, "RAW: 0 packed, 1 fp32 in place, 2 fp16 in place (fp16 engine), 3 features");
+    static_assert(CYC == 0 || (LR && !DUMP && LD >= 1 && LD <= CYC - 2 && CYC % 2 == 0), "compiled schedule: an LR kernel with an even cycle, its first LD layers' slots in LDS");
     if (p.gate != nullptr && __builtin_nontemporal_load(p.gate) == 0u) return;
 
     const int tid = threadIdx.x;
@@ -779,7 +782,7 @@
     char* const ringMine = (char*)p.ring + (size_t)tile0 * ringTile;
     const rsrc_t rsRing = make_rsrc(ringMine);
     const unsigned ringTileB = (unsigned)ringTile;
-    const int ldsD = LR ? p.ldsRingD : 0;
+    const int ldsD = CYC > 0 ? 1 << (LD > 0 ? LD - 1 : 0) : LR ? p.ldsRingD : 0;
     char* const ringLds = lds + C::ringSlotOffset(0, (int)C::ldsBytes(L, EMBLDS ? p.embLds : 0, DUMP));
     const char* condNext = condMine + (size_t)p.initSample * L * condStride;
     constexpr unsigned RAWE = RAW == 2 ? 2u : 4u;
@@ -787,8 +790,8 @@
     unsigned rawOff[BT];
 #pragma unroll
     for (int bt = 0; bt < BT; bt++) rawOff[bt] = ((unsigned)ub[bt] * (unsigned)(2 * R) + (unsigned)g * 4u) * RAWE;
-    auto prefetch = [&](int tn, int ln, Dil dl, frag (&xd)[BT][XPW], frag (&cdd)[BT][CR]) {
-        if (ln >= L) { ln -= L; tn += 1; }
+    auto prefetch = [&](int tn, int ln, auto wraps, const auto dl, frag (&xd)[BT][XPW], frag (&cdd)[BT][CR]) {
+        if (wraps) { ln -= L; tn += 1; }
         const unsigned slot = (unsigned)(dl.off + (tn & (dl.d - 1)));
         const unsigned rp0 = slot * (unsigned)(KF_R * 1024);
         const rsrc_t rsCond = make_rsrc(condNext);
@@ -849,9 +852,9 @@
         }
     };
     ring_lds_copy(std::true_type{});
-    prefetch(p.initSample, 0, p.dil[0], xpA, cdA);
-    prefetch(p.initSample, 1, p.dil[1], xpB, cdB);
-    auto publish_xp = [&](const frag (&xpN)[BT][XPW], const Dil dN) {
+    prefetch(p.initSample, 0, std::false_type{}, p.dil[0], xpA, cdA);
+    prefetch(p.initSample, 1, L <= 1, p.dil[1], xpB, cdB);
+    auto publish_xp = [&](const frag (&xpN)[BT][XPW], const auto dN) {
         if (dN.d <= ldsD) return;
 #pragma unroll
         for (int i = 0; i < XPW; i++) {
@@ -862,7 +865,7 @@
             }
         }
     };
-    auto tap_image = [&](const Dil dN, int tn) -> const char* {
+    auto tap_image = [&](const auto dN, int tn) -> const char* {
         return dN.d <= ldsD ? ringLds + (size_t)(dN.lds + (tn & (dN.d - 1))) * C::RING_SLOT : xpbuf;
     };
     publish_xp(xpA, p.dil[0]);
@@ -976,13 +979,13 @@
         frag xb[BT][KF_R];
 #pragma unroll
         for (int bt = 0; bt < BT; bt++) lds_get_frags<F16, KF_R>(xbuf + bt * KF_R * 1024, lane, xb[bt]);
-        auto layer = [&](auto withSkip, const int l, const Dil dl, const Dil dN, const Dil dl2, frag (&xpC)[BT][XPW],
+        auto layer = [&](auto withSkip, const int l, auto wrapN, auto wrap2, const auto dl, const auto dN, const auto dl2, frag (&xpC)[BT][XPW],
                          frag (&cdC)[BT][CR], const frag (&xpN)[BT][XPW], const frag (&cdN)[BT][CR]) {
             constexpr bool SKIP = decltype(withSkip)::value;
             constexpr int PB = SKIP ? 0 : FLW;
             const int wl = SKIP ? (l - 1) * FLW : 0;
             const float* bl = biasLds + l * BLS;
-            const int lN = l + 1 < L ? l + 1 : 0;
+            const int lN = wrapN ? 0 : l + 1;
             const float* blN = biasLds + lN * BLS;
             const int d = dl.d;
 
@@ -1008,7 +1011,7 @@
                         for (int bt = 0; bt < BT; bt++) xkeep[bt][k / NW] = xb[bt][k];
                     }
             }
-            if constexpr (!SKIP) prefetch(t, l + 2, dl2, xpC, cdC);
+            if constexpr (!SKIP) prefetch(t, l + 2, wrap2, dl2, xpC, cdC);
             __builtin_amdgcn_sched_barrier(0);
             WN_TMARK(2)
 
@@ -1061,7 +1064,7 @@
                     });
                     if constexpr (!EARLY || fi == NFS + NFC - 1) refill_group<F16, PF, 0, ws_pin, 1>(ws, rsW, pos, wl, 0, laneOff);
                     if constexpr (SKIP && fi == (NFS + NFC) * WN_REQ_AT_FEAT / 8) {
-                        prefetch(t, l + 2, dl2, xpC, cdC);
+                        prefetch(t, l + 2, wrap2, dl2, xpC, cdC);
                         __builtin_amdgcn_sched_barrier(0);
                     }
                 });
@@ -1120,7 +1123,7 @@
                         });
                         if constexpr (!EARLY || gi == STW * KF_R / G - 1) refill_group<F16, PF, 0, ws_pin, G>(ws, rsW, C::P_SKIP + gi * G, wl, 0, laneOff);
                         if constexpr (gi == (STW * KF_R / G) * WN_REQ_AT / 8) {
-                            prefetch(t, l + 2, dl2, xpC, cdC);
+                            prefetch(t, l + 2, wrap2, dl2, xpC, cdC);
                             __builtin_amdgcn_sched_barrier(0);
                         }
                     });
@@ -1207,7 +1210,7 @@
             wg_barrier();
             WN_TMARK(7)
             frag xp[BT][KF_R];
-            const char* const tapImg = tap_image(dN, l + 1 < L ? t : t + 1);
+            const char* const tapImg = tap_image(dN, wrapN ? t + 1 : t);
 #pragma unroll
             for (int bt = 0; bt < BT; bt++) lds_get_frags<F16, KF_R>(tapImg + bt * KF_R * 1024, lane, xp[bt]);
 #pragma unroll
@@ -1215,19 +1218,53 @@
             __builtin_amdgcn_sched_barrier(0);
             gemm_b<F16, PF, 0, BT, 2 * HTW, KF_R>(ws, rsW, C::P_PREV - PB, wl, 0, laneOff, acc, xp);
         };
-        {
+        if constexpr (CYC > 0) {
+            constexpr int SLOTS = (1 << CYC) - 1, LSLOTS = (1 << LD) - 1;
+            int ro = 0, lo = 0;
+            for (int c0 = 0; c0 < L; c0 += CYC) {
+                const bool last = c0 + CYC >= L;
+                const int roN = last ? 0 : ro + SLOTS, loN = last ? 0 : lo + LSLOTS;
+                static_for<CYC>([&](auto I) {
+                    constexpr int i = decltype(I)::value;
+                    auto entry = [&](auto J) {
+                        constexpr int jj = decltype(J)::value;
+                        if constexpr (jj < CYC) return DilC<jj, LD>(ro, lo);
+                        else return DilC<jj - CYC, LD>(roN, loN);
+                    };
+                    auto wraps = [&](auto J) {
+                        if constexpr (decltype(J)::value < CYC) return std::false_type{};
+                        else return last;
+                    };
+                    const auto dl = entry(I);
+                    const auto dN = entry(std::integral_constant<int, i + 1>{});
+                    const auto dl2 = entry(std::integral_constant<int, i + 2>{});
+                    const auto wrapN = wraps(std::integral_constant<int, i + 1>{});
+                    const auto wrap2 = wraps(std::integral_constant<int, i + 2>{});
+                    auto run = [&](auto withSkip) {
+                        if constexpr (i % 2 == 0) layer(withSkip, c0 + i, wrapN, wrap2, dl, dN, dl2, xpA, cdA, xpB, cdB);
+                        else layer(withSkip, c0 + i, wrapN, wrap2, dl, dN, dl2, xpB, cdB, xpA, cdA);
+                    };
+                    if constexpr (i == 0) {
+                        if (c0 == 0) run(std::false_type{});
+                        else run(std::true_type{});
+                    } else run(std::true_type{});
+                });
+                ro = roN;
+                lo = loN;
+            }
+        } else {
             Dil da = dil_first(), db = dil_next(da, p.maxDilation, L == 1, ldsD), dc = dil_next(db, p.maxDilation, L == 2, ldsD);
             auto adv = [&](int l) { da = db; db = dc; dc = dil_next(dc, p.maxDilation, l + 3 == L, ldsD); };
-            layer(std::false_type{}, 0, da, db, dc, xpA, cdA, xpB, cdB);
+            layer(std::false_type{}, 0, 1 >= L, 2 >= L, da, db, dc, xpA, cdA, xpB, cdB);
             adv(0);
             int l = 1;
             for (; l + 1 < L; l += 2) {
-                layer(std::true_type{}, l, da, db, dc, xpB, cdB, xpA, cdA);
+                layer(std::true_type{}, l, l + 1 >= L, l + 2 >= L, da, db, dc, xpB, cdB, xpA, cdA);
                 adv(l);
-                layer(std::true_type{}, l + 1, da, db, dc, xpA, cdA, xpB, cdB);
+                layer(std::true_type{}, l + 1, l + 2 >= L, l + 3 >= L, da, db, dc, xpA, cdA, xpB, cdB);
                 adv(l + 1);
             }
-            if (l < L) layer(std::true_type{}, l, da, db, dc, xpB, cdB, xpA, cdA);
+            if (l < L) layer(std::true_type{}, l, l + 1 >= L, l + 2 >= L, da, db, dc, xpB, cdB, xpA, cdA);
             if (L & 1) {
 #pragma unroll
                 for (int bt = 0; bt < BT; bt++) {
@@ -1414,6 +1451,18 @@
         p.clk[2] = __builtin_amdgcn_s_memtime();
         p.clk[3] = __builtin_amdgcn_s_memrealtime();
     }
+}
+template <bool F16, int R, int S, int A, int BT, bool EMBLDS, bool DUMP = true, int RAW = 0, bool LR = false>
+#ifdef WN_EXP_TWO_WG
+__global__ __launch_bounds__((Cfg<F16, R, S, A, BT>::THREADS), (BT == 1 ? 2 : 1)) void wavenet_wg(const Params p) {
+#else
+__global__ __launch_bounds__((Cfg<F16, R, S, A, BT>::THREADS), 1) void wavenet_wg(const Params p) {
+#endif
+    wavenet_wg_body<F16, R, S, A, BT, EMBLDS, DUMP, RAW, LR, 0, 0>(p);
+}
+template <bool F16, int R, int S, int A, int BT, bool EMBLDS, int CYC, int LD>
+__global__ __launch_bounds__((Cfg<F16, R, S, A, BT>::THREADS), 1) void wavenet_wg_cs(const Params p) {
+    wavenet_wg_body<F16, R, S, A, BT, EMBLDS, false, 0, true, CYC, LD>(p);
 }
 
 static __global__ void mulaw_pcm_kernel(const int* __restrict__ yOut, short* __restrict__ pcm,
diff --git a/nv_wavenet_amd/engine.py b/nv_wavenet_amd/engine.py
--- a/nv_wavenet_amd/engine.py
+++ b/nv_wavenet_amd/engine.py
@@ -279,6 +279,9 @@
 
     def setRingInLds(self, mode=0):
         lib.nvw_set_ring_in_lds(self._h, int(mode))
+
+    def setCompiledSchedule(self, mode=0):
+        lib.nvw_set_compiled_schedule(self._h, int(mode))
 
     def setClockProbe(self, on=True):
         lib.nvw_set_clock_probe(self._h, 1 if on else 0)
```

Result: faster. 333.3 million samples/s, median of 6 (+3.3%).
